# LariWa/Fractal-Image-Compression

Measured on NVIDIA B200. Metric: encode_evals_per_s, higher is better.
Workload: dtype u8

## Files before the change

### fractal-image-compression_b200/csrc/fic_search_umma.cu

```cuda
#include <cuda_fp16.h>

#include <cmath>
#include <mutex>
#include <tuple>
#include <vector>

#include "fic_device.cuh"

namespace fic {

namespace {

constexpr int kTileN = 128;
constexpr int kBlockM = 128;
constexpr int kAccs = 4;
constexpr int kRowsPerSB = kBlockM * kAccs;
constexpr int kEpiWarps = 16;
constexpr int kThreads = (4 + kEpiWarps) * 32;
constexpr int kChunksPerTile = kTileN / 32;
constexpr int kBoundBytes = kChunksPerTile * 2 * 4 + 16 + kChunksPerTile * 4;
constexpr int kNormOff = kChunksPerTile * 2 * 4 + 16;
constexpr int kFlagLists = 2;
constexpr int kFlagCap = 32;
constexpr float kOneMinusEps = 1.0f - 1.9073486328125e-06f;

template <int B, bool F16>
struct Cfg;
template <>
struct Cfg<8, false> {
    static constexpr int n = 64;
    static constexpr int NB = 4;
    static constexpr bool KSPLIT = false;
    static constexpr int KS_A = 3;
    static constexpr int KS_B = 5;
    static constexpr int NS = 5;
    static constexpr int NSTAGE = 7;
    __host__ __device__ static constexpr int amap(int s) { return s < 4 ? (s & 1) : 2; }
    __host__ __device__ static constexpr bool is_l_slice(int s) { return s == 2 || s == 3; }
};
template <>
struct Cfg<4, false> {
    static constexpr int n = 16;
    static constexpr int NB = 4;
    static constexpr bool KSPLIT = false;
    static constexpr int KS_A = 2;
    static constexpr int KS_B = 2;
    static constexpr int NS = 2;
    static constexpr int NSTAGE = 8;
    __host__ __device__ static constexpr int amap(int s) { return s; }
    __host__ __device__ static constexpr bool is_l_slice(int) { return false; }
};
template <>
struct Cfg<16, false> {
    static constexpr int n = 256;
    static constexpr int NB = 4;
    static constexpr bool KSPLIT = true;
    static constexpr int KS_P0 = 9, KS_P1 = 8;
    static constexpr int KS_A = 9;
    static constexpr int KS_B = 17;
    static constexpr int NS = 17;
    static constexpr int NSTAGE = 2;
    __host__ __device__ static constexpr int amap(int s) { return s < 16 ? (s & 7) : 8; }
    __host__ __device__ static constexpr bool is_l_slice(int s) { return s >= 8 && s < 16; }
};
template <>
struct Cfg<8, true> {
    static constexpr int n = 64;
    static constexpr int NB = 4;
    static constexpr bool KSPLIT = false;
    static constexpr int KS_A = 4;
    static constexpr int KS_B = 4;
    static constexpr int NS = 4;
    static constexpr int NSTAGE = 8;
    __host__ __device__ static constexpr int amap(int s) { return s; }
    __host__ __device__ static constexpr bool is_l_slice(int) { return false; }
};
template <>
struct Cfg<4, true> {
    static constexpr int n = 16;
    static constexpr int NB = 4;
    static constexpr bool KSPLIT = false;
    static constexpr int KS_A = 1;
    static constexpr int KS_B = 1;
    static constexpr int NS = 1;
    static constexpr int NSTAGE = 8;
    __host__ __device__ static constexpr int amap(int s) { return s; }
    __host__ __device__ static constexpr bool is_l_slice(int) { return false; }
};

template <>
struct Cfg<16, true> {
    static constexpr int n = 256;
    static constexpr int NB = 2;
    static constexpr bool KSPLIT = true;
    static constexpr int KS_P0 = 8, KS_P1 = 8;
    static constexpr int KS_A = 16;
    static constexpr int KS_B = 16;
    static constexpr int NS = 16;
    static constexpr int NSTAGE = 2;
    __host__ __device__ static constexpr int amap(int s) { return s; }
    __host__ __device__ static constexpr bool is_l_slice(int) { return false; }
};

template <class C>
constexpr int ksplit_p0()
{
    if constexpr (C::KSPLIT) return C::KS_P0;
    else return C::KS_B;
}

template <int B, bool F16>
struct Lay {
    using C = Cfg<B, F16>;
    static constexpr int SBO_A = C::KS_A * 256;
    static constexpr int A_BLOCK_BYTES = (kBlockM / 8) * SBO_A;
    static constexpr int ROWS_SB = C::NB * kBlockM;
    static constexpr int A_SB_BYTES = C::NB * A_BLOCK_BYTES;
    static constexpr int KS0 = ksplit_p0<C>();
    static constexpr int SBO_B = KS0 * 256;
    static constexpr int SBO_P1 = (C::KS_B - KS0) * 256;
    static constexpr int B_OP_BYTES = (kTileN / 8) * SBO_B;
    static constexpr int P0_BYTES = B_OP_BYTES + kBoundBytes;
    static constexpr int P1_BYTES = (kTileN / 8) * SBO_P1;
    static constexpr int B_TILE_BYTES = P0_BYTES + P1_BYTES;
    static constexpr int SLOT_BYTES = C::KSPLIT ? ((P0_BYTES + 127) / 128) * 128 : B_TILE_BYTES;
    static constexpr int PAIR_P0_BYTES = B_OP_BYTES / 2, PAIR_P1_BYTES = P1_BYTES / 2;
    static constexpr int PAIR_SLOT_BYTES = PAIR_P0_BYTES > PAIR_P1_BYTES ? PAIR_P0_BYTES : PAIR_P1_BYTES;
    static constexpr int PAIR_STAGES = (C::NSTAGE * SLOT_BYTES) / PAIR_SLOT_BYTES < 12 ? (C::NSTAGE * SLOT_BYTES) / PAIR_SLOT_BYTES : 12;
    static constexpr int BAR_BYTES = 512;
    static constexpr int SMEM_BYTES = A_SB_BYTES + C::NSTAGE * SLOT_BYTES + 1024  + BAR_BYTES  +
                                      kRowsPerSB * 4 ;
};

__device__ __noinline__ float flag_threshold(float lb, float tie_abs)
{
    const float rad = lb * lb * kOneMinusEps - tie_abs;
    return rad > 0.0f ? sqrtf(rad) : -1.0f;
}

struct RowFilter { float thresh, lbmax; int cnt; };
__device__ __noinline__ RowFilter flag_chunk(RowFilter st, float lb, float ub, float tie_abs, int2 *list, int chunk_id,
                                             uint32_t sh_lb, int share)
{
    if (st.cnt < kFlagCap) list[st.cnt] = make_int2(chunk_id, __float_as_int(ub));
    st.cnt++;
    if (lb > st.lbmax) {
        st.lbmax = lb;
        if (share)
            asm volatile("red.shared.max.u32 [%0], %1;" ::"r"(sh_lb), "r"(__float_as_uint(lb)) : "memory");
        const float rad = lb * lb * kOneMinusEps - tie_abs;
        st.thresh = rad > 0.0f ? sqrtf(rad) : -1.0f;
    }
    return st;
}


__host__ __device__ __forceinline__ int64_t sweep_to_sorted(int64_t pos, uint32_t mult, int64_t nch)
{
    const uint64_t chunk = (uint64_t)pos >> 5;
    return (int64_t)(((chunk * (uint64_t)mult) % (uint64_t)nch) * 32 + ((uint64_t)pos & 31));
}

__global__ void k_umma_sortkeys(const int32_t *__restrict__ dsum, const int32_t *__restrict__ dsq, int n,
                                int64_t ND, uint32_t *__restrict__ keys, int32_t *__restrict__ vals)
{
    int64_t j = (int64_t)blockIdx.x * blockDim.x + threadIdx.x;
    if (j >= ND) return;
    int dmean;
    keys[j] = (uint32_t)dom_var(dsum[j], dsq[j], n, &dmean);
    vals[j] = (int32_t)j;
}


constexpr int kSortSub = 512;

__global__ void __launch_bounds__(256) k_sort_hist(const uint32_t *__restrict__ keys, int64_t n, int shift, int64_t nwarps,
                                                   uint32_t *__restrict__ hist)
{
    __shared__ uint32_t s_h[8][256];
    const int warp = threadIdx.x >> 5, lane = threadIdx.x & 31;
    const int64_t gw = (int64_t)blockIdx.x * 8 + warp;
    for (int d = lane; d < 256; d += 32) s_h[warp][d] = 0;
    __syncwarp();
    if (gw < nwarps) {
        const int64_t a = gw * kSortSub, b = a + kSortSub < n ? a + kSortSub : n;
        for (int64_t i = a + lane; i < b; i += 32) atomicAdd(&s_h[warp][(keys[i] >> shift) & 255u], 1u);
        __syncwarp();
        for (int d = lane; d < 256; d += 32) hist[(int64_t)d * nwarps + gw] = s_h[warp][d];
    }
}

__global__ void __launch_bounds__(256) k_sort_scan_rows(uint32_t *__restrict__ hist, int64_t nwarps, uint32_t *__restrict__ totals)
{
    __shared__ uint32_t s_warp[8];
    __shared__ uint32_t s_carry;
    uint32_t *row = hist + (int64_t)blockIdx.x * nwarps;
    const int warp = threadIdx.x >> 5, lane = threadIdx.x & 31;
    if (threadIdx.x == 0) s_carry = 0;
    __syncthreads();
    for (int64_t base = 0; base < nwarps; base += 256) {
        const int64_t i = base + threadIdx.x;
        const uint32_t c = i < nwarps ? row[i] : 0u;
        uint32_t incl = c;
        for (int o = 1; o < 32; o <<= 1) {
            const uint32_t v = __shfl_up_sync(0xffffffffu, incl, o);
            if (lane >= o) incl += v;
        }
        if (lane == 31) s_warp[warp] = incl;
        __syncthreads();
        uint32_t before = s_carry;
        for (int w = 0; w < warp; w++) before += s_warp[w];
        if (i < nwarps) row[i] = before + incl - c;
        __syncthreads();
        if (threadIdx.x == 255) s_carry = before + incl;
        __syncthreads();
    }
    if (threadIdx.x == 0) totals[blockIdx.x] = s_carry;
}

__global__ void __launch_bounds__(256) k_sort_scatter(const uint32_t *__restrict__ keys, const int32_t *__restrict__ vals,
                                                      uint32_t *__restrict__ keys_out, int32_t *__restrict__ vals_out, int64_t n,
                                                      int shift, int64_t nwarps, const uint32_t *__restrict__ hist,
                                                      const uint32_t *__restrict__ totals)
{
    __shared__ uint32_t s_digit[256];
    __shared__ uint32_t s_base[8][256];
    const int warp = threadIdx.x >> 5, lane = threadIdx.x & 31;
    const int64_t gw = (int64_t)blockIdx.x * 8 + warp;
    {
        const uint32_t c = totals[threadIdx.x];
        uint32_t incl = c;
        for (int o = 1; o < 32; o <<= 1) {
            const uint32_t v = __shfl_up_sync(0xffffffffu, incl, o);
            if (lane >= o) incl += v;
        }
        s_digit[threadIdx.x] = incl - c;
        if (lane == 31) s_base[0][warp] = incl;
        __syncthreads();
        uint32_t before = 0;
        for (int w = 0; w < warp; w++) before += s_base[0][w];
        __syncthreads();
        s_digit[threadIdx.x] += before;
        __syncthreads();
    }
    if (gw >= nwarps) return;
    for (int d = lane; d < 256; d += 32) s_base[warp][d] = s_digit[d] + hist[(int64_t)d * nwarps + gw];
    __syncwarp();
    const int64_t a = gw * kSortSub, b = a + kSortSub < n ? a + kSortSub : n;
    for (int64_t i0 = a; i0 < b; i0 += 32) {
        const int64_t i = i0 + lane;
        const bool live = i < b;
        const uint32_t k = live ? keys[i] : 0u;
        const int32_t v = live ? vals[i] : 0;
        const uint32_t d = live ? ((k >> shift) & 255u) : 256u + lane;
        const unsigned peers = __match_any_sync(0xffffffffu, d);
        const int rank = __popc(peers & ((1u << lane) - 1u));
        uint32_t base = 0;
        if (live) base = s_base[warp][d];
        __syncwarp();
        if (live) {
            keys_out[base + rank] = k;
            vals_out[base + rank] = v;
            if (rank == 0) s_base[warp][d] = base + __popc(peers);
        }
        __syncwarp();
    }
}

inline size_t sort_hist_bytes(int64_t n) { return (size_t)256 * (size_t)((n + kSortSub - 1) / kSortSub + 1) * 4; }

inline int launch_sort_pairs(uint32_t *keys0, int32_t *vals0, uint32_t *keys1, int32_t *vals1, uint32_t *hist, int64_t n, cudaStream_t s)
{
    const int64_t nwarps = (n + kSortSub - 1) / kSortSub;
    const unsigned blocks = (unsigned)((nwarps + 7) / 8);
    uint32_t *totals = hist + 256 * nwarps;
    uint32_t *kin = keys0, *kout = keys1;
    int32_t *vin = vals0, *vout = vals1;
    for (int pass = 0; pass < 3; pass++) {
        k_sort_hist<<<blocks, 256, 0, s>>>(kin, n, 8 * pass, nwarps, hist);
        k_sort_scan_rows<<<256, 256, 0, s>>>(hist, nwarps, totals);
        k_sort_scatter<<<blocks, 256, 0, s>>>(kin, vin, kout, vout, n, 8 * pass, nwarps, hist, totals);
        uint32_t *tk = kin; kin = kout; kout = tk;
        int32_t *tv = vin; vin = vout; vout = tv;
    }
    return 9;
}


__device__ __forceinline__ uint32_t pack4(int a, int b, int c, int d)
{
    return (uint32_t)(a & 0xff) | ((uint32_t)(b & 0xff) << 8) | ((uint32_t)(c & 0xff) << 16) | ((uint32_t)(d & 0xff) << 24);
}

template <int n>
__host__ __device__ __forceinline__ int64_t raw_offset(int64_t pos, int c)
{
    return (pos >> 5) * (32 * n) + c * 512 + (pos & 31) * 16;
}

__device__ __forceinline__ uint32_t pack_h2(int lo, int hi)
{
    const __half2 v = __halves2half2(__int2half_rn(lo), __int2half_rn(hi));
    return *(const uint32_t *)&v;
}

template <int B, bool F16>
__global__ void __launch_bounds__(128)
k_umma_pack_domains(const uint8_t *__restrict__ dec, const int32_t *__restrict__ dsum,
                    const int32_t *__restrict__ dsq, const int32_t *__restrict__ perm, uint8_t *__restrict__ opB,
                    int32_t *__restrict__ pos_dom, int4 *__restrict__ pos_info,
                    uint8_t *__restrict__ pos_raw, int64_t *__restrict__ dom0_pos,
                    Geom g, int64_t ntiles, uint32_t mult)
{
    using L = Lay<B, F16>;
    constexpr int n = Cfg<B, F16>::n;
    const int64_t pos = (int64_t)blockIdx.x * blockDim.x + threadIdx.x;
    const int64_t tile = pos / kTileN;
    const int row = (int)(pos % kTileN);
    const int64_t sp = sweep_to_sorted(pos, mult, ntiles * kChunksPerTile);
    constexpr bool KSPLIT = Cfg<B, F16>::KSPLIT;
    uint8_t *blob = opB + tile * L::B_TILE_BYTES;
    uint8_t *rowp = blob + (row >> 3) * L::SBO_B + (row & 7) * 16;
    uint8_t *rowp1 = blob + L::P0_BYTES + (row >> 3) * L::SBO_P1 + (row & 7) * 16;
    constexpr int NCH = L::KS0 * 2;
    constexpr int NCH1 = (Cfg<B, F16>::KS_B - L::KS0) * 2;
    float rsd_hi = 0.0f, rsd_lo = __int_as_float(0x7f800000);
    int any_l = 0;
    if (sp >= g.ND) {
#pragma unroll
        for (int c = 0; c < NCH; c++) *(uint4 *)(rowp + c * 128) = make_uint4(0, 0, 0, 0);
#pragma unroll
        for (int c = 0; c < NCH1; c++) *(uint4 *)(rowp1 + c * 128) = make_uint4(0, 0, 0, 0);
        pos_dom[pos] = -1;
        pos_info[pos] = make_int4(-1, 0, 0, 0);
    } else {
        const int64_t j = perm[sp];
        const int gx = (int)(j % g.dpw), gy = (int)(j / g.dpw);
        const uint8_t *p = dec + (int64_t)(gy * g.step) * g.sw + gx * g.step;
        int dmean;
        const int varD = dom_var(dsum[j], dsq[j], n, &dmean);
        constexpr int PCH = n / 16;
        const int sgn = (!F16 && dmean == 0) ? -1 : 1;
        const bool wide8 = B == 8 && (g.sw & 7) == 0;
        const int col8 = (gx * g.step) & 7;
#pragma unroll
        for (int c = 0; c < PCH; c++) {
            int dv[16];
            uint32_t raw[4];
            if (wide8) {
#pragma unroll
                for (int r2 = 0; r2 < 2; r2++) {
                    const uint8_t *q = p + (int64_t)(c * 2 + r2) * g.sw - col8;
                    const uint2 lo = __ldg((const uint2 *)q);
                    uint2 hi = lo;
                    if (col8) hi = __ldg((const uint2 *)(q + 8));
                    const uint32_t sh = (uint32_t)(col8 & 3) * 8u;
                    const bool up = col8 >= 4;
                    raw[2 * r2] = __funnelshift_r(up ? lo.y : lo.x, up ? hi.x : lo.y, sh);
                    raw[2 * r2 + 1] = __funnelshift_r(up ? hi.x : lo.y, up ? hi.y : hi.x, sh);
                }
            }
#pragma unroll
            for (int w = 0; w < 4; w++) {
                const int k = c * 16 + w * 4;
                const uint8_t *q = p + (int64_t)(k / B) * g.sw + (k % B);
                if (B == 16) raw[w] = __ldg((const uint32_t *)q);
                else if (B == 8) {
                    if (!wide8) raw[w] = (uint32_t)__ldg((const uint16_t *)q) | ((uint32_t)__ldg((const uint16_t *)(q + 2)) << 16);
                } else raw[w] = (uint32_t)__ldg(q) | ((uint32_t)__ldg(q + 1) << 8) | ((uint32_t)__ldg(q + 2) << 16) | ((uint32_t)__ldg(q + 3) << 24);
#pragma unroll
                for (int e = 0; e < 4; e++) dv[w * 4 + e] = sgn * ((int)((raw[w] >> (8 * e)) & 0xffu) - dmean);
            }
            *(uint4 *)(pos_raw + raw_offset<n>(pos, c)) = make_uint4(raw[0], raw[1], raw[2], raw[3]);
            if (F16) {
                *(uint4 *)(rowp + (2 * c) * 128) =
                    make_uint4(pack_h2(dv[0], dv[1]), pack_h2(dv[2], dv[3]), pack_h2(dv[4], dv[5]), pack_h2(dv[6], dv[7]));
                *(uint4 *)(rowp + (2 * c + 1) * 128) = make_uint4(pack_h2(dv[8], dv[9]), pack_h2(dv[10], dv[11]),
                                                                  pack_h2(dv[12], dv[13]), pack_h2(dv[14], dv[15]));
            } else {
                uint32_t hw[4], lw[4];
#pragma unroll
                for (int w = 0; w < 4; w++) {
                    int hv[4], lv[4];
#pragma unroll
                    for (int e = 0; e < 4; e++) {
                        hv[e] = max(-128, min(127, dv[w * 4 + e]));
                        lv[e] = dv[w * 4 + e] - hv[e];
                        any_l |= lv[e];
                    }
                    hw[w] = pack4(hv[0], hv[1], hv[2], hv[3]);
                    lw[w] = pack4(lv[0], lv[1], lv[2], lv[3]);
                }
                *(uint4 *)(rowp + c * 128) = make_uint4(hw[0], hw[1], hw[2], hw[3]);
                if (KSPLIT) *(uint4 *)(rowp1 + c * 128) = make_uint4(lw[0], lw[1], lw[2], lw[3]);
                else *(uint4 *)(rowp + (PCH + c) * 128) = make_uint4(lw[0], lw[1], lw[2], lw[3]);
            }
        }
        if (!F16) {
            const int alpha = sgn * (dsum[j] - n * dmean);
            const int a1 = alpha / 3, a2 = (alpha - a1) / 2, a3 = alpha - a1 - a2;
            constexpr int ACH = KSPLIT ? PCH : 2 * PCH;
            *(uint4 *)(rowp + ACH * 128) = make_uint4(
                (uint32_t)((-a1) & 0xff) | ((uint32_t)((-a2) & 0xff) << 8) | ((uint32_t)((-a3) & 0xff) << 16), 0, 0, 0);
            *(uint4 *)(rowp + (ACH + 1) * 128) = make_uint4(0, 0, 0, 0);
        }
        pos_dom[pos] = (int32_t)j;
        pos_info[pos] = make_int4((int32_t)j, varD, dsum[j], 0);
        if (j == 0) *dom0_pos = pos;
        if (varD > 0) {
            float r = __double2float_rn(__ddiv_rn(1.0, __dsqrt_rn((double)varD)));
            rsd_hi = r * (1.0f + 4.76837158203125e-07f);
            rsd_lo = r * (1.0f - 4.76837158203125e-07f);
        }
    }
    for (int o = 16; o > 0; o >>= 1) {
        rsd_hi = fmaxf(rsd_hi, __shfl_xor_sync(0xffffffffu, rsd_hi, o));
        rsd_lo = fminf(rsd_lo, __shfl_xor_sync(0xffffffffu, rsd_lo, o));
    }
    if ((threadIdx.x & 31) == 0) {
        if (rsd_hi == 0.0f) rsd_lo = 0.0f;
        *(float2 *)(blob + L::B_OP_BYTES + (row >> 5) * 8) = make_float2(rsd_hi, rsd_lo);
    }
    const int tile_has_l = __syncthreads_or(any_l != 0);
    if (threadIdx.x == 0) *(uint4 *)(blob + L::B_OP_BYTES + kChunksPerTile * 8) = make_uint4((uint32_t)tile_has_l, 0, 0, 0);
}

template <int B, bool F16>
__global__ void __launch_bounds__(128)
k_umma_pack_ranges(const uint8_t *__restrict__ src, const int32_t *__restrict__ rsum, uint8_t *__restrict__ opA,
                   int32_t *__restrict__ vRout, Geom g, int64_t j0, int64_t j1, int64_t rows_padded)
{
    using L = Lay<B, F16>;
    constexpr int n = Cfg<B, F16>::n;
    int64_t i = (int64_t)blockIdx.x * blockDim.x + threadIdx.x;
    if (i >= rows_padded) return;
    int64_t sb = i / L::ROWS_SB;
    int rr = (int)(i % L::ROWS_SB);
    int blk = rr / kBlockM, row = rr % kBlockM;
    uint8_t *rowp = opA + sb * L::A_SB_BYTES + blk * L::A_BLOCK_BYTES + (row >> 3) * L::SBO_A + (row & 7) * 16;
    constexpr int NCH = Cfg<B, F16>::KS_A * 2;
    const int64_t j = j0 + i / g.n_iso;
    const int kiso = (int)(i % g.n_iso);
    if (j >= j1) {
#pragma unroll
        for (int c = 0; c < NCH; c++) *(uint4 *)(rowp + c * 128) = make_uint4(0, 0, 0, 0);
        vRout[i] = 0;
        return;
    }
    int xr = (int)(j % g.rpw), yr = (int)(j / g.rpw);
    const uint8_t *p = src + (int64_t)(yr * B) * g.W + xr * B;
    int rmean;
    vRout[i] = centred_sum(rsum[j], n, &rmean);
    constexpr int PCH = n / 16;
#pragma unroll
    for (int c = 0; c < PCH; c++) {
        uint32_t w4[4];
#pragma unroll
        for (int w = 0; w < 4; w++) {
            int k = c * 16 + w * 4;
            if (kiso == 0) {
                w4[w] = *(const uint32_t *)(p + (int64_t)(k / B) * g.W + (k % B));
            } else {
                w4[w] = 0;
#pragma unroll
                for (int e = 0; e < 4; e++) {
                    int ry, rx;
                    iso_map(iso_inverse(kiso), B, (k + e) / B, (k + e) % B, &ry, &rx);
                    w4[w] |= (uint32_t)p[(int64_t)ry * g.W + rx] << (8 * e);
                }
            }
        }
        if (F16) {
            uint32_t hw[8];
#pragma unroll
            for (int w = 0; w < 4; w++) {
                hw[2 * w] = pack_h2((int)(w4[w] & 0xff) - rmean, (int)((w4[w] >> 8) & 0xff) - rmean);
                hw[2 * w + 1] = pack_h2((int)((w4[w] >> 16) & 0xff) - rmean, (int)(w4[w] >> 24) - rmean);
            }
            *(uint4 *)(rowp + (2 * c) * 128) = make_uint4(hw[0], hw[1], hw[2], hw[3]);
            *(uint4 *)(rowp + (2 * c + 1) * 128) = make_uint4(hw[4], hw[5], hw[6], hw[7]);
        } else {
            uint4 v = make_uint4(w4[0], w4[1], w4[2], w4[3]);
            *(uint4 *)(rowp + c * 128) = v;
            if (B == 4) *(uint4 *)(rowp + (PCH + c) * 128) = v;
        }
    }
    if (!F16) {
        constexpr int XCH = (B == 4) ? 2 * PCH : PCH;
        *(uint4 *)(rowp + XCH * 128) = make_uint4((uint32_t)rmean | ((uint32_t)rmean << 8) | ((uint32_t)rmean << 16), 0, 0, 0);
        *(uint4 *)(rowp + (XCH + 1) * 128) = make_uint4(0, 0, 0, 0);
    }
}


__global__ void k_umma_sortkeys_rgb(const int32_t *__restrict__ dsum, int n, int64_t ND, uint32_t *__restrict__ keys,
                                    int32_t *__restrict__ vals)
{
    int64_t j = (int64_t)blockIdx.x * blockDim.x + threadIdx.x;
    if (j >= ND) return;
    int dm[3];
    const int vd = centred_sum_rgb(dsum, ND, j, n, dm);
    keys[j] = (uint32_t)(vd * vd);
    vals[j] = (int32_t)j;
}

template <int B>
__device__ __forceinline__ uint8_t *rgb_dom_piece(uint8_t *blob, int row, int c)
{
    using L = Lay<B, true>;
    constexpr int NCH0 = L::KS0 * 2;
    if (!Cfg<B, true>::KSPLIT || c < NCH0) return blob + (row >> 3) * L::SBO_B + (row & 7) * 16 + c * 128;
    return blob + L::P0_BYTES + (row >> 3) * L::SBO_P1 + (row & 7) * 16 + (c - NCH0) * 128;
}

template <int B>
__global__ void __launch_bounds__(128)
k_umma_pack_domains_rgb(const uint16_t *__restrict__ dec3, const int32_t *__restrict__ dsum,
                        const int32_t *__restrict__ perm, uint8_t *__restrict__ opB, int32_t *__restrict__ pos_dom,
                        int4 *__restrict__ pos_info, int64_t *__restrict__ dom0_pos, Geom g, int64_t ntiles, uint32_t mult)
{
    using L = Lay<B, true>;
    constexpr int n = B * B;
    const int64_t pos = (int64_t)blockIdx.x * blockDim.x + threadIdx.x;
    const int64_t tile = pos / kTileN;
    const int row = (int)(pos % kTileN);
    const int64_t sp = sweep_to_sorted(pos, mult, ntiles * kChunksPerTile);
    uint8_t *blob = opB + tile * L::B_TILE_BYTES;
    constexpr int NCH = n / 8;
    float rsd_hi = 0.0f, rsd_lo = __int_as_float(0x7f800000), norm = 0.0f;
    if (sp >= g.ND) {
#pragma unroll
        for (int c = 0; c < NCH; c++) *(uint4 *)rgb_dom_piece<B>(blob, row, c) = make_uint4(0, 0, 0, 0);
        pos_dom[pos] = -1;
        pos_info[pos] = make_int4(-1, 0, 0, 0);
    } else {
        const int64_t j = perm[sp];
        const int gx = (int)(j % g.dpw), gy = (int)(j / g.dpw);
        const uint16_t *p = dec3 + (int64_t)(gy * g.step) * g.sw + gx * g.step;
        int dm[3];
        const int vd = centred_sum_rgb(dsum, g.ND, j, n, dm);
        const int dmsum = dm[0] + dm[1] + dm[2];
        uint32_t sumsq = 0;
#pragma unroll
        for (int c = 0; c < NCH; c++) {
            int dv[8];
            const int k0 = c * 8;
            const uint16_t *q = p + (int64_t)(k0 / B) * g.sw + (k0 % B);
            if (B == 16) {
#pragma unroll
                for (int e = 0; e < 8; e += 4) {
                    const uint2 w = __ldg((const uint2 *)(q + e));
                    dv[e] = (int)(w.x & 0xffffu); dv[e + 1] = (int)(w.x >> 16);
                    dv[e + 2] = (int)(w.y & 0xffffu); dv[e + 3] = (int)(w.y >> 16);
                }
            } else if (B == 8) {
#pragma unroll
                for (int e = 0; e < 8; e += 2) {
                    const uint32_t w = __ldg((const uint32_t *)(q + e));
                    dv[e] = (int)(w & 0xffffu);
                    dv[e + 1] = (int)(w >> 16);
                }
            } else {
#pragma unroll
                for (int e = 0; e < 8; e++) {
                    const int k = k0 + e;
                    dv[e] = (int)__ldg(p + (int64_t)(k / B) * g.sw + (k % B));
                }
            }
#pragma unroll
            for (int e = 0; e < 8; e++) {
                dv[e] = vd != 0 ? dv[e] - dmsum : 0;
                sumsq += (uint32_t)(dv[e] * dv[e]);
            }
            *(uint4 *)rgb_dom_piece<B>(blob, row, c) =
                make_uint4(pack_h2(dv[0], dv[1]), pack_h2(dv[2], dv[3]), pack_h2(dv[4], dv[5]), pack_h2(dv[6], dv[7]));
        }
        pos_dom[pos] = (int32_t)j;
        pos_info[pos] = make_int4((int32_t)j, vd, 0, 0);
        if (j == 0) *dom0_pos = pos;
        if (vd > 0) {
            float r = __double2float_rn(__ddiv_rn(1.0, (double)vd));
            rsd_hi = r * (1.0f + 4.76837158203125e-07f);
            rsd_lo = r * (1.0f - 4.76837158203125e-07f);
        }
        norm = __fsqrt_ru((float)sumsq) * (1.0f + 2.384185791015625e-07f);
    }
    for (int o = 16; o > 0; o >>= 1) {
        rsd_hi = fmaxf(rsd_hi, __shfl_xor_sync(0xffffffffu, rsd_hi, o));
        rsd_lo = fminf(rsd_lo, __shfl_xor_sync(0xffffffffu, rsd_lo, o));
        norm = fmaxf(norm, __shfl_xor_sync(0xffffffffu, norm, o));
    }
    if ((threadIdx.x & 31) == 0) {
        if (rsd_hi == 0.0f) rsd_lo = 0.0f;
        *(float2 *)(blob + L::B_OP_BYTES + (row >> 5) * 8) = make_float2(rsd_hi, rsd_lo);
        *(float *)(blob + L::B_OP_BYTES + kNormOff + (row >> 5) * 4) = norm;
    }
    if (threadIdx.x == 0) *(uint4 *)(blob + L::B_OP_BYTES + kChunksPerTile * 8) = make_uint4(Cfg<B, true>::KSPLIT ? 1u : 0u, 0, 0, 0);
}

template <int B>
__global__ void __launch_bounds__(128)
k_umma_pack_ranges_rgb(const uint8_t *__restrict__ src, const int32_t *__restrict__ rsum, uint8_t *__restrict__ opA,
                       int32_t *__restrict__ vRout, float *__restrict__ nRout, Geom g, int64_t j0, int64_t j1, int64_t rows_padded)
{
    using L = Lay<B, true>;
    constexpr int n = B * B;
    int64_t i = (int64_t)blockIdx.x * blockDim.x + threadIdx.x;
    if (i >= rows_padded) return;
    int64_t sb = i / L::ROWS_SB;
    int rr = (int)(i % L::ROWS_SB);
    int blk = rr / kBlockM, row = rr % kBlockM;
    uint8_t *rowp = opA + sb * L::A_SB_BYTES + blk * L::A_BLOCK_BYTES + (row >> 3) * L::SBO_A + (row & 7) * 16;
    constexpr int NCH = n / 8;
    const int64_t j = j0 + i;
    if (j >= j1) {
#pragma unroll
        for (int c = 0; c < NCH; c++) *(uint4 *)(rowp + c * 128) = make_uint4(0, 0, 0, 0);
        vRout[i] = 0;
        if (nRout) nRout[i] = 0.0f;
        return;
    }
    const int xr = (int)(j % g.rpw), yr = (int)(j / g.rpw);
    const int64_t plane = (int64_t)g.W * g.H;
    const uint8_t *p = src + (int64_t)(yr * B) * g.W + xr * B;
    int rm[3];
    const int vR = centred_sum_rgb(rsum, g.NR, j, n, rm);
    const int rmsum = rm[0] + rm[1] + rm[2];
    uint32_t sumsq = 0;
#pragma unroll
    for (int c = 0; c < NCH; c++) {
        int rv[8];
#pragma unroll
        for (int e = 0; e < 8; e++) {
            const int k = c * 8 + e;
            const uint8_t *q = p + (int64_t)(k / B) * g.W + (k % B);
            rv[e] = (int)q[0] + (int)q[plane] + (int)q[2 * plane] - rmsum;
            sumsq += (uint32_t)(rv[e] * rv[e]);
        }
        *(uint4 *)(rowp + c * 128) =
            make_uint4(pack_h2(rv[0], rv[1]), pack_h2(rv[2], rv[3]), pack_h2(rv[4], rv[5]), pack_h2(rv[6], rv[7]));
    }
    vRout[i] = vR;
    if (nRout) nRout[i] = __fsqrt_ru((float)sumsq) * (1.0f + 2.384185791015625e-07f);
}


__device__ __forceinline__ uint32_t smem_u32(const void *p) { return (uint32_t)__cvta_generic_to_shared(p); }

__device__ __forceinline__ void mbar_init(uint32_t bar, uint32_t count)
{
    asm volatile("mbarrier.init.shared::cta.b64 [%0], %1;" ::"r"(bar), "r"(count));
}
__device__ __forceinline__ void mbar_arrive(uint32_t bar)
{
    asm volatile("mbarrier.arrive.shared::cta.b64 _, [%0];" ::"r"(bar) : "memory");
}
__device__ __forceinline__ void mbar_expect_tx(uint32_t bar, uint32_t bytes)
{
    asm volatile("mbarrier.arrive.expect_tx.shared::cta.b64 _, [%0], %1;" ::"r"(bar), "r"(bytes) : "memory");
}
__device__ __forceinline__ uint32_t mbar_try_wait(uint32_t bar, uint32_t parity)
{
    uint32_t ok;
    asm volatile(
        "{\n\t.reg .pred p;\n\t"
        "mbarrier.try_wait.parity.shared::cta.b64 p, [%1], %2;\n\t"
        "selp.u32 %0, 1, 0, p;\n\t}"
        : "=r"(ok)
        : "r"(bar), "r"(parity)
        : "memory");
    return ok;
}
__device__ __noinline__ void mbar_timeout(volatile int *status, int code)
{
    if (status) {
        *status = code;
        __threadfence_system();
    }
    __trap();
}
__device__ __noinline__ void mbar_wait_slow(uint32_t bar, uint32_t parity, volatile int *status, int code)
{
    long long t0 = clock64();
    while (!mbar_try_wait(bar, parity)) {
        if (clock64() - t0 > 2000000000ll) mbar_timeout(status, code);
    }
}
__device__ __forceinline__ void mbar_wait(uint32_t bar, uint32_t parity, volatile int *status, int code)
{
    if (mbar_try_wait(bar, parity)) return;
    mbar_wait_slow(bar, parity, status, code);
}
__device__ __forceinline__ void bulk_g2s(uint32_t dst, const void *src, uint32_t bytes, uint32_t bar)
{
    asm volatile("cp.async.bulk.shared::cluster.global.mbarrier::complete_tx::bytes [%0], [%1], %2, [%3];" ::"r"(dst),
                 "l"(src), "r"(bytes), "r"(bar)
                 : "memory");
}
__device__ __forceinline__ uint32_t elect_one()
{
    uint32_t pred;
    asm volatile(
        "{\n\t.reg .pred p;\n\t.reg .b32 r;\n\t"
        "elect.sync r|p, 0xffffffff;\n\t"
        "selp.u32 %0, 1, 0, p;\n\t}"
        : "=r"(pred));
    return pred;
}
__device__ __forceinline__ void tc_fence_before() { asm volatile("tcgen05.fence::before_thread_sync;" ::: "memory"); }
__device__ __forceinline__ void tc_fence_after() { asm volatile("tcgen05.fence::after_thread_sync;" ::: "memory"); }
__device__ __forceinline__ void tc_commit(uint32_t bar)
{
    asm volatile("tcgen05.commit.cta_group::1.mbarrier::arrive::one.shared::cluster.b64 [%0];" ::"r"(bar) : "memory");
}
__device__ __forceinline__ void tc_mma_i8(uint32_t d_tmem, uint64_t adesc, uint64_t bdesc, uint32_t idesc, uint32_t acc)
{
    asm volatile(
        "{\n\t.reg .pred p;\n\tsetp.ne.b32 p, %4, 0;\n\t"
        "tcgen05.mma.cta_group::1.kind::i8 [%0], %1, %2, %3, p;\n\t}" ::"r"(d_tmem),
        "l"(adesc), "l"(bdesc), "r"(idesc), "r"(acc)
        : "memory");
}
__device__ __forceinline__ void tc_mma_f16(uint32_t d_tmem, uint64_t adesc, uint64_t bdesc, uint32_t idesc, uint32_t acc)
{
    asm volatile(
        "{\n\t.reg .pred p;\n\tsetp.ne.b32 p, %4, 0;\n\t"
        "tcgen05.mma.cta_group::1.kind::f16 [%0], %1, %2, %3, p;\n\t}" ::"r"(d_tmem),
        "l"(adesc), "l"(bdesc), "r"(idesc), "r"(acc)
        : "memory");
}
__device__ __forceinline__ uint32_t cluster_ctarank()
{
    uint32_t r;
    asm volatile("mov.u32 %0, %%cluster_ctarank;" : "=r"(r));
    return r;
}
__device__ __forceinline__ void cluster_sync_all()
{
    asm volatile("barrier.cluster.arrive.release.aligned;\n\tbarrier.cluster.wait.acquire.aligned;" ::: "memory");
}
__device__ __forceinline__ uint32_t mapa_u32(uint32_t saddr, uint32_t rank)
{
    uint32_t r;
    asm volatile("mapa.shared::cluster.u32 %0, %1, %2;" : "=r"(r) : "r"(saddr), "r"(rank));
    return r;
}
__device__ __forceinline__ void mbar_arrive_cluster(uint32_t cluster_addr)
{
    asm volatile("mbarrier.arrive.shared::cluster.b64 _, [%0];" ::"r"(cluster_addr) : "memory");
}
__device__ __forceinline__ void tc_commit2(uint32_t bar, uint32_t mask)
{
    asm volatile("tcgen05.commit.cta_group::2.mbarrier::arrive::one.shared::cluster.multicast::cluster.b64 [%0], %1;" ::"r"(bar),
                 "h"((uint16_t)mask)
                 : "memory");
}
__device__ __forceinline__ void tc_mma2_i8(uint32_t d_tmem, uint64_t adesc, uint64_t bdesc, uint32_t idesc, uint32_t acc)
{
    asm volatile(
        "{\n\t.reg .pred p;\n\tsetp.ne.b32 p, %4, 0;\n\t"
        "tcgen05.mma.cta_group::2.kind::i8 [%0], %1, %2, %3, p;\n\t}" ::"r"(d_tmem),
        "l"(adesc), "l"(bdesc), "r"(idesc), "r"(acc)
        : "memory");
}
__device__ __forceinline__ void tc_mma2_f16(uint32_t d_tmem, uint64_t adesc, uint64_t bdesc, uint32_t idesc, uint32_t acc)
{
    asm volatile(
        "{\n\t.reg .pred p;\n\tsetp.ne.b32 p, %4, 0;\n\t"
        "tcgen05.mma.cta_group::2.kind::f16 [%0], %1, %2, %3, p;\n\t}" ::"r"(d_tmem),
        "l"(adesc), "l"(bdesc), "r"(idesc), "r"(acc)
        : "memory");
}
__device__ __forceinline__ void tmem_ld32(uint32_t taddr, uint32_t (&v)[32])
{
    asm volatile(
        "tcgen05.ld.sync.aligned.32x32b.x32.b32 "
        "{%0, %1, %2, %3, %4, %5, %6, %7, %8, %9, %10, %11, %12, %13, %14, %15, "
        "%16, %17, %18, %19, %20, %21, %22, %23, %24, %25, %26, %27, %28, %29, %30, %31}, [%32];"
        : "=r"(v[0]), "=r"(v[1]), "=r"(v[2]), "=r"(v[3]), "=r"(v[4]), "=r"(v[5]), "=r"(v[6]), "=r"(v[7]),
          "=r"(v[8]), "=r"(v[9]), "=r"(v[10]), "=r"(v[11]), "=r"(v[12]), "=r"(v[13]), "=r"(v[14]), "=r"(v[15]),
          "=r"(v[16]), "=r"(v[17]), "=r"(v[18]), "=r"(v[19]), "=r"(v[20]), "=r"(v[21]), "=r"(v[22]), "=r"(v[23]),
          "=r"(v[24]), "=r"(v[25]), "=r"(v[26]), "=r"(v[27]), "=r"(v[28]), "=r"(v[29]), "=r"(v[30]), "=r"(v[31])
        : "r"(taddr)
        : "memory");
}
__device__ __forceinline__ void sts_u32(uint32_t saddr, uint32_t v)
{
    asm volatile("st.shared.u32 [%0], %1;" ::"r"(saddr), "r"(v) : "memory");
}
__device__ __forceinline__ uint32_t lds_volatile_u32(uint32_t saddr)
{
    uint32_t v;
    asm volatile("ld.volatile.shared.u32 %0, [%1];" : "=r"(v) : "r"(saddr) : "memory");
    return v;
}
__device__ __forceinline__ void pin_order(uint32_t (&v)[32])
{
    asm volatile(""
                 : "+r"(v[0]), "+r"(v[1]), "+r"(v[2]), "+r"(v[3]), "+r"(v[4]), "+r"(v[5]), "+r"(v[6]), "+r"(v[7]), "+r"(v[8]),
                   "+r"(v[9]), "+r"(v[10]), "+r"(v[11]), "+r"(v[12]), "+r"(v[13]), "+r"(v[14]), "+r"(v[15]), "+r"(v[16]),
                   "+r"(v[17]), "+r"(v[18]), "+r"(v[19]), "+r"(v[20]), "+r"(v[21]), "+r"(v[22]), "+r"(v[23]), "+r"(v[24]),
                   "+r"(v[25]), "+r"(v[26]), "+r"(v[27]), "+r"(v[28]), "+r"(v[29]), "+r"(v[30]), "+r"(v[31])
                 :
                 : "memory");
}
__device__ __forceinline__ void tmem_ld_wait() { asm volatile("tcgen05.wait::ld.sync.aligned;" ::: "memory"); }
__device__ __forceinline__ int dp4a_uu(uint32_t a_u8x4, uint32_t b_u8x4, int c)
{
    int d;
    asm("dp4a.u32.u32 %0, %1, %2, %3;" : "=r"(d) : "r"(a_u8x4), "r"(b_u8x4), "r"(c));
    return d;
}

__device__ __forceinline__ uint64_t make_desc(uint32_t saddr, uint32_t lbo_bytes, uint32_t sbo_bytes)
{
    return (uint64_t)((saddr >> 4) & 0x3fff) | ((uint64_t)((lbo_bytes >> 4) & 0x3fff) << 16) |
           ((uint64_t)((sbo_bytes >> 4) & 0x3fff) << 32) | ((uint64_t)1 << 46);
}

constexpr uint32_t kIdesc = (2u << 4) | (0u << 7) | (1u << 10) | ((uint32_t)(kTileN >> 3) << 17) |
                            ((uint32_t)(kBlockM >> 4) << 24);
constexpr uint32_t kIdescF16 = (1u << 4) | (0u << 7) | (0u << 10) | ((uint32_t)(kTileN >> 3) << 17) |
                               ((uint32_t)(kBlockM >> 4) << 24);
constexpr uint32_t kIdescPair = (2u << 4) | (0u << 7) | (1u << 10) | ((uint32_t)(kTileN >> 3) << 17) |
                                ((uint32_t)((2 * kBlockM) >> 4) << 24);
constexpr uint32_t kIdescF16Pair = (1u << 4) | (0u << 7) | (0u << 10) | ((uint32_t)(kTileN >> 3) << 17) |
                                   ((uint32_t)((2 * kBlockM) >> 4) << 24);


template <int B, bool F16, bool PAIR>
__host__ __device__ constexpr int epi_of() { return (!F16 || B == 16) ? 0 : ((B == 4 || PAIR) ? 3 : 2); }

template <int B, bool F16, bool PAIR, bool DUMP>
__global__ void __launch_bounds__(kThreads, 1)
k_umma_search(const uint8_t *__restrict__ opA, const uint8_t *__restrict__ opB, const int32_t *__restrict__ vRarr,
              const float *__restrict__ nRarr, int2 *__restrict__ flag_list, int32_t *__restrict__ flag_cnt, uint32_t *__restrict__ row_lb, int n_sb,
              int n_chunks, int ntiles, int iso_shift, int64_t rows_padded, int32_t *__restrict__ dump, int64_t dump_ld, volatile int *status)
{
    using C = Cfg<B, F16>;
    using L = Lay<B, F16>;
    static_assert(!PAIR || F16 || C::KSPLIT, "CTA pairs: kind::f16, or the K-split configurations (B = 16)");
    constexpr int EPI = DUMP ? 0 : epi_of<B, F16, PAIR>();
    constexpr int NISS = (PAIR && !C::KSPLIT) ? 2 : 1;
    constexpr int NSTAGE = PAIR ? L::PAIR_STAGES : C::NSTAGE;
    constexpr int SLOT = PAIR ? L::PAIR_SLOT_BYTES : L::SLOT_BYTES;
    extern __shared__ __align__(1024) uint8_t smem_raw[];
    uint8_t *smem = (uint8_t *)(((uintptr_t)smem_raw + 1023) & ~(uintptr_t)1023);
    uint8_t *sA = smem;
    uint8_t *sB = smem + L::A_SB_BYTES;
    uint64_t *bars = (uint64_t *)(sB + C::NSTAGE * L::SLOT_BYTES);
    uint32_t bar0 = smem_u32(bars);
    asm volatile("" : "+r"(bar0));
    auto BAR_B_FULL = [&](int s) { return bar0 + 8u * s; };
    auto BAR_B_EMPTY = [&](int s) { return bar0 + 8u * (NSTAGE + s); };
    auto BAR_T_FULL = [&](int q) { return bar0 + 8u * (2 * NSTAGE + q); };
    auto BAR_T_EMPTY = [&](int q) { return bar0 + 8u * (2 * NSTAGE + kAccs + q); };
    const uint32_t BAR_A_FULL = bar0 + 8u * (2 * NSTAGE + 2 * kAccs);
    const uint32_t BAR_A_EMPTY = BAR_A_FULL + 8u;
    uint32_t *tmem_slot = (uint32_t *)(bars + 2 * NSTAGE + 2 * kAccs + 2);
    const uint32_t s_has_l = bar0 + 400u;
    uint32_t *s_lb = (uint32_t *)((uint8_t *)bars + L::BAR_BYTES);

    const int warp = threadIdx.x >> 5, lane = threadIdx.x & 31;
    const uint32_t rank = PAIR ? cluster_ctarank() : 0u;
    const int u_first = PAIR ? (int)(blockIdx.x >> 1) : (int)blockIdx.x, u_step = PAIR ? (int)(gridDim.x >> 1) : (int)gridDim.x;
    const int n_sbu = PAIR ? (n_sb >> 1) : n_sb;

    if (warp == 1 && lane == 0) {
        const uint32_t both = (PAIR && rank == 0) ? 2u : 1u;
        for (int s = 0; s < NSTAGE; s++) {
            mbar_init(BAR_B_FULL(s), both);
            mbar_init(BAR_B_EMPTY(s), NISS);
        }
        for (int q = 0; q < kAccs; q++) {
            mbar_init(BAR_T_FULL(q), 1);
            mbar_init(BAR_T_EMPTY(q), both * (kEpiWarps / kAccs));
        }
        mbar_init(BAR_A_FULL, both);
        mbar_init(BAR_A_EMPTY, NISS);
        asm volatile("fence.mbarrier_init.release.cluster;" ::: "memory");
    }
    if (warp == 2) {
        if (PAIR) {
            asm volatile("tcgen05.alloc.cta_group::2.sync.aligned.shared::cta.b32 [%0], %1;" ::"r"(smem_u32(tmem_slot)), "r"(512u) : "memory");
            asm volatile("tcgen05.relinquish_alloc_permit.cta_group::2.sync.aligned;" ::: "memory");
        } else {
            asm volatile("tcgen05.alloc.cta_group::1.sync.aligned.shared::cta.b32 [%0], %1;" ::"r"(smem_u32(tmem_slot)), "r"(512u) : "memory");
            asm volatile("tcgen05.relinquish_alloc_permit.cta_group::1.sync.aligned;" ::: "memory");
        }
    }
    tc_fence_before();
    if (PAIR) cluster_sync_all();
    else __syncthreads();
    tc_fence_after();
    const uint32_t tmem_base = *tmem_slot;

    const int n_units = n_sbu * n_chunks;

    if (warp == 0) {
        if (lane == 0) {
            uint32_t stage = 0, phase = 0, a_phase = 0;
            for (int u = u_first; u < n_units; u += u_step) {
                int sb = PAIR ? 2 * (u % n_sbu) + (int)rank : u % n_sbu, ch = u / n_sbu;
                int t0 = (int)((int64_t)ch * ntiles / n_chunks), t1 = (int)((int64_t)(ch + 1) * ntiles / n_chunks);
                mbar_wait(BAR_A_EMPTY, a_phase ^ 1, status, 1);
                mbar_expect_tx(BAR_A_FULL, L::A_SB_BYTES);
                bulk_g2s(smem_u32(sA), opA + (int64_t)sb * L::A_SB_BYTES, L::A_SB_BYTES, BAR_A_FULL);
                for (int t = t0; t < t1; t++) {
                    const uint8_t *blob = opB + (int64_t)t * L::B_TILE_BYTES;
                    if (C::KSPLIT && PAIR) {
                        const uint32_t has_l = __ldg((const uint32_t *)(blob + L::B_OP_BYTES + kChunksPerTile * 8));
                        mbar_wait(BAR_B_EMPTY(stage), phase ^ 1, status, 2);
                        sts_u32(s_has_l + 4u * stage, has_l);
                        mbar_expect_tx(BAR_B_FULL(stage), L::PAIR_P0_BYTES);
                        bulk_g2s(smem_u32(sB + stage * SLOT), blob + rank * L::PAIR_P0_BYTES, L::PAIR_P0_BYTES, BAR_B_FULL(stage));
                        if (++stage == NSTAGE) { stage = 0; phase ^= 1; }
                        if (has_l) {
                            mbar_wait(BAR_B_EMPTY(stage), phase ^ 1, status, 2);
                            mbar_expect_tx(BAR_B_FULL(stage), L::PAIR_P1_BYTES);
                            bulk_g2s(smem_u32(sB + stage * SLOT), blob + L::P0_BYTES + rank * L::PAIR_P1_BYTES, L::PAIR_P1_BYTES, BAR_B_FULL(stage));
                            if (++stage == NSTAGE) { stage = 0; phase ^= 1; }
                        }
                    } else if (C::KSPLIT) {
                        mbar_wait(BAR_B_EMPTY(stage), phase ^ 1, status, 2);
                        mbar_expect_tx(BAR_B_FULL(stage), L::P0_BYTES);
                        bulk_g2s(smem_u32(sB + stage * L::SLOT_BYTES), blob, L::P0_BYTES, BAR_B_FULL(stage));
                        if (++stage == NSTAGE) { stage = 0; phase ^= 1; }
                        const uint32_t has_l = __ldg((const uint32_t *)(blob + L::B_OP_BYTES + kChunksPerTile * 8));
                        if (has_l) {
                            mbar_wait(BAR_B_EMPTY(stage), phase ^ 1, status, 2);
                            mbar_expect_tx(BAR_B_FULL(stage), L::P1_BYTES);
                            bulk_g2s(smem_u32(sB + stage * L::SLOT_BYTES), blob + L::P0_BYTES, L::P1_BYTES, BAR_B_FULL(stage));
                            if (++stage == NSTAGE) { stage = 0; phase ^= 1; }
                        }
                    } else if (PAIR) {
                        mbar_wait(BAR_B_EMPTY(stage), phase ^ 1, status, 2);
                        mbar_expect_tx(BAR_B_FULL(stage), SLOT);
                        bulk_g2s(smem_u32(sB + stage * SLOT), blob + rank * SLOT, SLOT, BAR_B_FULL(stage));
                        if (++stage == NSTAGE) { stage = 0; phase ^= 1; }
                    } else {
                        mbar_wait(BAR_B_EMPTY(stage), phase ^ 1, status, 2);
                        mbar_expect_tx(BAR_B_FULL(stage), L::B_TILE_BYTES);
                        bulk_g2s(smem_u32(sB + stage * L::SLOT_BYTES), blob, L::B_TILE_BYTES, BAR_B_FULL(stage));
                        if (++stage == NSTAGE) { stage = 0; phase ^= 1; }
                    }
                }
                a_phase ^= 1;
            }
        }
        __syncwarp();
    } else if (PAIR && (warp == 1 || (warp == 3 && !C::KSPLIT))) {
        if constexpr (PAIR && C::KSPLIT) {
            if (rank == 0) {
                uint32_t stage = 0, phase = 0, a_phase = 0, t_phase = 0;
                const uint32_t elected = elect_one();
                const uint64_t a_desc0 = make_desc(smem_u32(sA), 128, L::SBO_A);
                for (int u = u_first; u < n_units; u += u_step) {
                    int ch = u / n_sbu;
                    int t0 = (int)((int64_t)ch * ntiles / n_chunks), t1 = (int)((int64_t)(ch + 1) * ntiles / n_chunks);
                    mbar_wait(BAR_A_FULL, a_phase, status, 3);
                    for (int t = t0; t < t1; t++) {
                        mbar_wait(BAR_B_FULL(stage), phase, status, 4);
                        tc_fence_after();
                        const uint32_t has_l = lds_volatile_u32(s_has_l + 4u * stage);
                        const uint64_t b0 = make_desc(smem_u32(sB + stage * SLOT), 128, L::SBO_B);
#pragma unroll
                        for (int q = 0; q < C::NB; q++) {
                            mbar_wait(BAR_T_EMPTY(q), ((t_phase >> q) & 1) ^ 1, status, 5);
                            tc_fence_after();
                            if (elected) {
#pragma unroll
                                for (int s = 0; s < L::KS0; s++) {
                                    const uint64_t ad = a_desc0 + (uint64_t)((q * L::A_BLOCK_BYTES + s * 256) >> 4);
                                    if (F16) tc_mma2_f16(tmem_base + q * kTileN, ad, b0 + (uint64_t)((s * 256) >> 4), kIdescF16Pair, s > 0 ? 1u : 0u);
                                    else tc_mma2_i8(tmem_base + q * kTileN, ad, b0 + (uint64_t)((s * 256) >> 4), kIdescPair, s > 0 ? 1u : 0u);
                                }
                                if (!has_l) tc_commit2(BAR_T_FULL(q), 3u);
                            }
                            __syncwarp();
                            t_phase ^= 1u << q;
                        }
                        if (elected) tc_commit2(BAR_B_EMPTY(stage), 3u);
                        __syncwarp();
                        if (++stage == NSTAGE) { stage = 0; phase ^= 1; }
                        if (has_l) {
                            mbar_wait(BAR_B_FULL(stage), phase, status, 4);
                            tc_fence_after();
                            const uint64_t b1 = make_desc(smem_u32(sB + stage * SLOT), 128, L::SBO_P1);
#pragma unroll
                            for (int q = 0; q < C::NB; q++) {
                                if (elected) {
#pragma unroll
                                    for (int s = 0; s < C::KS_B - L::KS0; s++) {
                                        const int sa = F16 ? L::KS0 + s : s;
                                        const uint64_t ad = a_desc0 + (uint64_t)((q * L::A_BLOCK_BYTES + sa * 256) >> 4);
                                        if (F16) tc_mma2_f16(tmem_base + q * kTileN, ad, b1 + (uint64_t)((s * 256) >> 4), kIdescF16Pair, 1u);
                                        else tc_mma2_i8(tmem_base + q * kTileN, ad, b1 + (uint64_t)((s * 256) >> 4), kIdescPair, 1u);
                                    }
                                    tc_commit2(BAR_T_FULL(q), 3u);
                                }
                                __syncwarp();
                            }
                            if (elected) tc_commit2(BAR_B_EMPTY(stage), 3u);
                            __syncwarp();
                            if (++stage == NSTAGE) { stage = 0; phase ^= 1; }
                        }
                    }
                    if (elected) tc_commit2(BAR_A_EMPTY, 3u);
                    __syncwarp();
                    a_phase ^= 1;
                }
            } else {
                if (lane == 0) {
                    uint32_t stage = 0, phase = 0, a_phase = 0;
                    const uint32_t ra_full = mapa_u32(BAR_A_FULL, 0);
                    for (int u = u_first; u < n_units; u += u_step) {
                        int ch = u / n_sbu;
                        int t0 = (int)((int64_t)ch * ntiles / n_chunks), t1 = (int)((int64_t)(ch + 1) * ntiles / n_chunks);
                        mbar_wait(BAR_A_FULL, a_phase, status, 3);
                        mbar_arrive_cluster(ra_full);
                        for (int t = t0; t < t1; t++) {
                            mbar_wait(BAR_B_FULL(stage), phase, status, 4);
                            const uint32_t has_l = lds_volatile_u32(s_has_l + 4u * stage);
                            mbar_arrive_cluster(mapa_u32(BAR_B_FULL(stage), 0));
                            if (++stage == NSTAGE) { stage = 0; phase ^= 1; }
                            if (has_l) {
                                mbar_wait(BAR_B_FULL(stage), phase, status, 4);
                                mbar_arrive_cluster(mapa_u32(BAR_B_FULL(stage), 0));
                                if (++stage == NSTAGE) { stage = 0; phase ^= 1; }
                            }
                        }
                        a_phase ^= 1;
                    }
                }
                __syncwarp();
            }
        } else if constexpr (PAIR) {
            if (rank == 0) {
                const int qi = warp >> 1;
                uint32_t stage = 0, phase = 0, a_phase = 0, t_phase = 0;
                const uint32_t elected = elect_one();
                const uint64_t a_desc0 = make_desc(smem_u32(sA), 128, L::SBO_A);
                const uint64_t b_desc0 = make_desc(smem_u32(sB), 128, L::SBO_B);
                for (int u = u_first; u < n_units; u += u_step) {
                    int ch = u / n_sbu;
                    int t0 = (int)((int64_t)ch * ntiles / n_chunks), t1 = (int)((int64_t)(ch + 1) * ntiles / n_chunks);
                    mbar_wait(BAR_A_FULL, a_phase, status, 3);
                    for (int t = t0; t < t1; t++) {
                        mbar_wait(BAR_B_FULL(stage), phase, status, 4);
                        tc_fence_after();
                        const uint64_t b_desc = b_desc0 + (uint64_t)((stage * SLOT) >> 4);
#pragma unroll
                        for (int k = 0; k < 2; k++) {
                            const int q = qi + 2 * k;
                            mbar_wait(BAR_T_EMPTY(q), ((t_phase >> k) & 1) ^ 1, status, 5);
                            tc_fence_after();
                            if (elected) {
#pragma unroll
                                for (int s = 0; s < C::NS; s++) {
                                    const uint64_t ad = a_desc0 + (uint64_t)((q * L::A_BLOCK_BYTES + C::amap(s) * 256) >> 4);
                                    tc_mma2_f16(tmem_base + q * kTileN, ad, b_desc + (uint64_t)((s * 256) >> 4), kIdescF16Pair, s > 0 ? 1u : 0u);
                                }
                                tc_commit2(BAR_T_FULL(q), 3u);
                                if (k == 1) tc_commit2(BAR_B_EMPTY(stage), 3u);
                            }
                            __syncwarp();
                            t_phase ^= 1u << k;
                        }
                        if (++stage == NSTAGE) { stage = 0; phase ^= 1; }
                    }
                    if (elected) tc_commit2(BAR_A_EMPTY, 3u);
                    __syncwarp();
                    a_phase ^= 1;
                }
            } else if (warp == 1) {
                if (lane == 0) {
                    uint32_t stage = 0, phase = 0, a_phase = 0;
                    const uint32_t ra_full = mapa_u32(BAR_A_FULL, 0);
                    for (int u = u_first; u < n_units; u += u_step) {
                        int ch = u / n_sbu;
                        int t0 = (int)((int64_t)ch * ntiles / n_chunks), t1 = (int)((int64_t)(ch + 1) * ntiles / n_chunks);
                        mbar_wait(BAR_A_FULL, a_phase, status, 3);
                        mbar_arrive_cluster(ra_full);
                        for (int t = t0; t < t1; t++) {
                            mbar_wait(BAR_B_FULL(stage), phase, status, 4);
                            mbar_arrive_cluster(mapa_u32(BAR_B_FULL(stage), 0));
                            if (++stage == NSTAGE) { stage = 0; phase ^= 1; }
                        }
                        a_phase ^= 1;
                    }
                }
                __syncwarp();
            }
        }
    } else if (warp == 1) {
        uint32_t stage = 0, phase = 0, a_phase = 0, t_phase = 0;
        const uint32_t elected = elect_one();
        const uint64_t a_desc0 = make_desc(smem_u32(sA), 128, L::SBO_A);
        const uint64_t b_desc0 = make_desc(smem_u32(sB), 128, L::SBO_B);
        for (int u = u_first; u < n_units; u += u_step) {
            int ch = u / n_sbu;
            int t0 = (int)((int64_t)ch * ntiles / n_chunks), t1 = (int)((int64_t)(ch + 1) * ntiles / n_chunks);
            mbar_wait(BAR_A_FULL, a_phase, status, 3);
            for (int t = t0; t < t1; t++) {
                mbar_wait(BAR_B_FULL(stage), phase, status, 4);
                tc_fence_after();
                const uint32_t has_l = *(volatile const uint32_t *)(sB + stage * L::SLOT_BYTES + L::B_OP_BYTES + kChunksPerTile * 8);
                if (C::KSPLIT) {
                    const uint64_t b0 = make_desc(smem_u32(sB + stage * L::SLOT_BYTES), 128, L::SBO_B);
#pragma unroll
                    for (int q = 0; q < C::NB; q++) {
                        mbar_wait(BAR_T_EMPTY(q), ((t_phase >> q) & 1) ^ 1, status, 5);
                        tc_fence_after();
                        if (elected) {
#pragma unroll
                            for (int s = 0; s < L::KS0; s++) {
                                const uint64_t ad = a_desc0 + (uint64_t)((q * L::A_BLOCK_BYTES + s * 256) >> 4);
                                if (F16) tc_mma_f16(tmem_base + q * kTileN, ad, b0 + (uint64_t)((s * 256) >> 4), kIdescF16, s > 0 ? 1u : 0u);
                                else tc_mma_i8(tmem_base + q * kTileN, ad, b0 + (uint64_t)((s * 256) >> 4), kIdesc, s > 0 ? 1u : 0u);
                            }
                            if (!has_l) tc_commit(BAR_T_FULL(q));
                        }
                        __syncwarp();
                        t_phase ^= 1u << q;
                    }
                    if (elected) tc_commit(BAR_B_EMPTY(stage));
                    __syncwarp();
                    if (++stage == NSTAGE) { stage = 0; phase ^= 1; }
                    if (has_l) {
                        mbar_wait(BAR_B_FULL(stage), phase, status, 4);
                        tc_fence_after();
                        const uint64_t b1 = make_desc(smem_u32(sB + stage * L::SLOT_BYTES), 128, L::SBO_P1);
#pragma unroll
                        for (int q = 0; q < C::NB; q++) {
                            if (elected) {
#pragma unroll
                                for (int s = 0; s < C::KS_B - L::KS0; s++) {
                                    const int sa = F16 ? L::KS0 + s : s;
                                    const uint64_t ad = a_desc0 + (uint64_t)((q * L::A_BLOCK_BYTES + sa * 256) >> 4);
                                    if (F16) tc_mma_f16(tmem_base + q * kTileN, ad, b1 + (uint64_t)((s * 256) >> 4), kIdescF16, 1u);
                                    else tc_mma_i8(tmem_base + q * kTileN, ad, b1 + (uint64_t)((s * 256) >> 4), kIdesc, 1u);
                                }
                                tc_commit(BAR_T_FULL(q));
                            }
                            __syncwarp();
                        }
                        if (elected) tc_commit(BAR_B_EMPTY(stage));
                        __syncwarp();
                        if (++stage == NSTAGE) { stage = 0; phase ^= 1; }
                    }
                    continue;
                }
                const uint64_t b_desc = b_desc0 + (uint64_t)((stage * L::SLOT_BYTES) >> 4);
#pragma unroll
                for (int q = 0; q < C::NB; q++) {
                    mbar_wait(BAR_T_EMPTY(q), ((t_phase >> q) & 1) ^ 1, status, 5);
                    tc_fence_after();
                    if (elected) {
#pragma unroll
                        for (int s = 0; s < C::NS; s++) {
                            if (C::is_l_slice(s) && !has_l) continue;
                            const uint64_t ad = a_desc0 + (uint64_t)((q * L::A_BLOCK_BYTES + C::amap(s) * 256) >> 4);
                            const uint64_t bd = b_desc + (uint64_t)((s * 256) >> 4);
                            if (F16) tc_mma_f16(tmem_base + q * kTileN, ad, bd, kIdescF16, s > 0 ? 1u : 0u);
                            else tc_mma_i8(tmem_base + q * kTileN, ad, bd, kIdesc, s > 0 ? 1u : 0u);
                        }
                        tc_commit(BAR_T_FULL(q));
                    }
                    __syncwarp();
                    t_phase ^= 1u << q;
                }
                if (elected) tc_commit(BAR_B_EMPTY(stage));
                __syncwarp();
                if (++stage == NSTAGE) { stage = 0; phase ^= 1; }
            }
            if (elected) tc_commit(BAR_A_EMPTY);
            __syncwarp();
            a_phase ^= 1;
        }
    } else if (warp >= 4) {
        const int e = warp - 4;
        const int lq = e & 3, q = e >> 2;
        const uint32_t ta = tmem_base + ((uint32_t)(lq * 32) << 16) + q * kTileN;
        uint32_t tf_phase = 0;
        const uint32_t bar_hand_back = PAIR ? mapa_u32(BAR_T_EMPTY(q), 0) : BAR_T_EMPTY(q);
        auto hand_back = [&]() {
            if (PAIR) mbar_arrive_cluster(bar_hand_back);
            else mbar_arrive(bar_hand_back);
        };
        constexpr bool SLACK = B == 16 && F16;
        const int n_units_mine = q < C::NB ? n_units : 0;
        for (int u = u_first; u < n_units_mine; u += u_step) {
            int sb = PAIR ? 2 * (u % n_sbu) + (int)rank : u % n_sbu, ch = u / n_sbu;
            int t0 = (int)((int64_t)ch * ntiles / n_chunks), t1 = (int)((int64_t)(ch + 1) * ntiles / n_chunks);
            const int64_t row = (int64_t)sb * L::ROWS_SB + q * kBlockM + lq * 32 + lane;
            const int vR = vRarr[row];
            const float nR = SLACK ? nRarr[row] : 0.0f;
            RowFilter st;
            st.thresh = (vR == 0) ? __int_as_float(0x7f800000) : -1.0f;
            st.lbmax = 0.0f;
            st.cnt = 0;
            const float tie_abs = (float)(vR * vR) * 4.76837158203125e-07f;
            const uint32_t sh_lb = smem_u32(s_lb + q * kBlockM + (((lq * 32 + lane) >> iso_shift) << iso_shift));
            if (iso_shift) {
                sts_u32(sh_lb, 0u);
                __syncwarp();
            }
            if (ch > 0 && vR != 0) {
                const float seed = __uint_as_float(*(volatile const uint32_t *)(row_lb + ((row >> iso_shift) << iso_shift)));
                if (seed > 0.0f) {
                    st.lbmax = seed;
                    st.thresh = flag_threshold(seed, tie_abs);
                }
            }
            int2 *const list0 = flag_list + (((int64_t)ch * rows_padded + row) * kFlagLists) * kFlagCap;
            int cnt0 = 0, cnt1 = 0;
            for (int t = t0; t < t1; t++) {
                const float4 *gb = (const float4 *)(opB + (int64_t)t * L::B_TILE_BYTES + L::B_OP_BYTES);
                const float4 bnd01 = __ldg(gb), bnd23 = __ldg(gb + 1);
                float4 bndn = make_float4(0.0f, 0.0f, 0.0f, 0.0f);
                if (SLACK) bndn = __ldg(gb + 3);
                mbar_wait(BAR_T_FULL(q), tf_phase, status, 7);
                tc_fence_after();
                if (iso_shift) {
                    const float other = __uint_as_float(lds_volatile_u32(sh_lb));
                    if (other > st.lbmax) {
                        st.lbmax = other;
                        st.thresh = flag_threshold(other, tie_abs);
                    }
                }
                if constexpr (EPI != 0) {
                    uint32_t v[32];
                    float Mc[kChunksPerTile];
                    tmem_ld32(ta, v);
                    tmem_ld_wait();
                    pin_order(v);
                    auto test = [&](int c) {
                        const float rhi = c == 0 ? bnd01.x : (c == 1 ? bnd01.z : (c == 2 ? bnd23.x : bnd23.z));
                        const float rlo = c == 0 ? bnd01.y : (c == 1 ? bnd01.w : (c == 2 ? bnd23.y : bnd23.w));
                        const float ub = Mc[c] * rhi;
                        if (ub > st.thresh) {
                            st.cnt = c < 2 ? cnt0 : cnt1;
                            st = flag_chunk(st, Mc[c] * rlo, ub, tie_abs, list0 + (c >> 1) * kFlagCap, t * kChunksPerTile + c, sh_lb, iso_shift ? 1 : 0);
                            if (c < 2) cnt0 = st.cnt;
                            else cnt1 = st.cnt;
                        }
                    };
#pragma unroll
                    for (int c = 0; c < kChunksPerTile; c++) {
                        auto av = [&](int k) { return fabsf(__uint_as_float(v[k])); };
                        float l[11];
#pragma unroll
                        for (int i = 0; i < 10; i++) l[i] = fmaxf(fmaxf(av(3 * i), av(3 * i + 1)), av(3 * i + 2));
                        l[10] = fmaxf(av(30), av(31));
                        if (c + 1 < kChunksPerTile) {
                            uint32_t next = ta + (c + 1) * 32;
                            asm volatile("" : "+r"(next) : "f"(l[0]), "f"(l[1]), "f"(l[2]), "f"(l[3]), "f"(l[4]), "f"(l[5]), "f"(l[6]),
                                         "f"(l[7]), "f"(l[8]), "f"(l[9]), "f"(l[10]));
                            tmem_ld32(next, v);
                        }
                        asm volatile("" : "+f"(l[0]), "+f"(l[1]), "+f"(l[2]), "+f"(l[3]), "+f"(l[4]), "+f"(l[5]), "+f"(l[6]), "+f"(l[7]),
                                     "+f"(l[8]), "+f"(l[9]), "+f"(l[10]));
                        const float m0 = fmaxf(fmaxf(l[0], l[1]), l[2]), m1 = fmaxf(fmaxf(l[3], l[4]), l[5]);
                        const float m2 = fmaxf(fmaxf(l[6], l[7]), l[8]), m3 = fmaxf(fmaxf(l[9], l[10]), m0);
                        Mc[c] = fmaxf(fmaxf(m1, m2), m3);
                        if (EPI == 2) test(c);
                        if (c + 1 < kChunksPerTile) {
                            tmem_ld_wait();
                            pin_order(v);
                            if (c + 1 == kChunksPerTile - 1) {
                                tc_fence_before();
                                __syncwarp();
                                if (lane == 0) hand_back();
                                if (EPI == 3) {
                                    asm volatile("" : "+f"(Mc[0]), "+f"(Mc[1]), "+f"(Mc[2]) : : "memory");
                                    test(0);
                                    test(1);
                                    test(2);
                                }
                            }
                        }
                    }
                    if (EPI == 3) test(kChunksPerTile - 1);
                } else {
#pragma unroll
                for (int c = 0; c < kChunksPerTile; c++) {
                    uint32_t v[32];
                    tmem_ld32(ta + c * 32, v);
                    tmem_ld_wait();
                    if (c == kChunksPerTile - 1) {
                        tc_fence_before();
                        __syncwarp();
                        if (lane == 0) hand_back();
                    }
                    float M;
                    if (F16) {
                        auto av = [&](int k) { return fabsf(__uint_as_float(v[k])); };
                        float c4[4];
#pragma unroll
                        for (int i = 0; i < 4; i++) {
                            c4[i] = fmaxf(fmaxf(av(8 * i), av(8 * i + 1)), av(8 * i + 2));
                            c4[i] = fmaxf(c4[i], fmaxf(av(8 * i + 3), av(8 * i + 4)));
                            c4[i] = fmaxf(c4[i], fmaxf(av(8 * i + 5), av(8 * i + 6)));
                        }
                        const float m01 = fmaxf(fmaxf(c4[0], c4[1]), av(7));
                        const float m23 = fmaxf(fmaxf(c4[2], c4[3]), av(15));
                        M = fmaxf(fmaxf(fmaxf(m01, m23), av(23)), av(31));
                    } else {
                        int mx0 = 0, mn0 = 0, mx1 = 0, mn1 = 0;
#pragma unroll
                        for (int k = 0; k < 32; k += 4) {
                            mx0 = max(mx0, max((int)v[k], (int)v[k + 1]));
                            mn0 = min(mn0, min((int)v[k], (int)v[k + 1]));
                            mx1 = max(mx1, max((int)v[k + 2], (int)v[k + 3]));
                            mn1 = min(mn1, min((int)v[k + 2], (int)v[k + 3]));
                        }
                        M = __int2float_rn(max(max(mx0, mx1), -min(mn0, mn1)));
                    }
                    if (DUMP) {
#pragma unroll
                        for (int k = 0; k < 32; k++) {
                            int iv = (int)v[k];
                            if (F16) {
                                const float f = __uint_as_float(v[k]);
                                iv = (f == rintf(f) && fabsf(f) < 2.0e9f) ? (int)f : (int)0x80000000;
                            }
                            dump[row * dump_ld + (int64_t)t * kTileN + c * 32 + k] = iv;
                        }
                    }
                    const float rhi = c == 0 ? bnd01.x : (c == 1 ? bnd01.z : (c == 2 ? bnd23.x : bnd23.z));
                    const float rlo = c == 0 ? bnd01.y : (c == 1 ? bnd01.w : (c == 2 ? bnd23.y : bnd23.w));
                    float Mu = M, Ml = M;
                    if (SLACK) {
                        const float pn = nR * (c == 0 ? bndn.x : (c == 1 ? bndn.y : (c == 2 ? bndn.z : bndn.w)));
                        if (pn >= 16777216.0f) {
                            const float sl = pn * 6.0e-5f;
                            Mu = M + sl;
                            Ml = fmaxf(M - sl, 0.0f);
                        }
                    }
                    const float ub = Mu * rhi;
                    if (ub > st.thresh) {
                        st.cnt = c < 2 ? cnt0 : cnt1;
                        st = flag_chunk(st, Ml * rlo, ub, tie_abs, list0 + (c >> 1) * kFlagCap, t * kChunksPerTile + c, sh_lb, iso_shift ? 1 : 0);
                        if (c < 2) cnt0 = st.cnt;
                        else cnt1 = st.cnt;
                    }
                }
                }
                tf_phase ^= 1;
            }
            flag_cnt[((int64_t)ch * rows_padded + row) * 2] = cnt0;
            flag_cnt[((int64_t)ch * rows_padded + row) * 2 + 1] = cnt1;
            if (st.lbmax > 0.0f) atomicMax(row_lb + ((row >> iso_shift) << iso_shift), __float_as_uint(st.lbmax));
        }
    }

    tc_fence_before();
    if (PAIR) cluster_sync_all();
    else __syncthreads();
    if (warp == 2) {
        tc_fence_after();
        if (PAIR) asm volatile("tcgen05.dealloc.cta_group::2.sync.aligned.b32 %0, %1;" ::"r"(tmem_base), "r"(512u) : "memory");
        else asm volatile("tcgen05.dealloc.cta_group::1.sync.aligned.b32 %0, %1;" ::"r"(tmem_base), "r"(512u) : "memory");
    }
}


template <bool F16, int N>
__global__ void __launch_bounds__(128, 1) k_mma_peak(int iters, uint32_t seed)
{
    extern __shared__ __align__(1024) uint8_t smem_raw[];
    uint8_t *smem = (uint8_t *)(((uintptr_t)smem_raw + 1023) & ~(uintptr_t)1023);
    uint8_t *sA = smem;
    uint8_t *sB = smem + 4096;
    uint64_t *bar = (uint64_t *)(smem + 4096 + 8192);
    uint32_t *tmem_slot = (uint32_t *)(bar + 1);
    const int warp = threadIdx.x >> 5;
    for (int i = threadIdx.x; i < (4096 + 8192) / 4; i += blockDim.x) {
        uint32_t x = (uint32_t)i * 2654435761u + seed + blockIdx.x * 40503u;
        x ^= x >> 15; x *= 0x2c1b3c6du; x ^= x >> 12;
        if (F16) x &= 0x3fff3fffu;
        ((uint32_t *)smem)[i] = x;
    }
    if (threadIdx.x == 0) {
        mbar_init(smem_u32(bar), 1);
        asm volatile("fence.mbarrier_init.release.cluster;" ::: "memory");
    }
    asm volatile("fence.proxy.async.shared::cta;" ::: "memory");
    if (warp == 0) {
        asm volatile("tcgen05.alloc.cta_group::1.sync.aligned.shared::cta.b32 [%0], %1;" ::"r"(smem_u32(tmem_slot)),
                     "r"(512u)
                     : "memory");
        asm volatile("tcgen05.relinquish_alloc_permit.cta_group::1.sync.aligned;" ::: "memory");
    }
    tc_fence_before();
    __syncthreads();
    tc_fence_after();
    const uint32_t tmem_base = *tmem_slot;
    if (warp == 1) {
        const uint32_t elected = elect_one();
        const uint64_t ad = make_desc(smem_u32(sA), 128, 256);
        const uint64_t bd = make_desc(smem_u32(sB), 128, 256);
        constexpr uint32_t idesc = (F16 ? ((1u << 4) | (0u << 7) | (0u << 10)) : ((2u << 4) | (0u << 7) | (1u << 10))) |
                                   ((uint32_t)(N >> 3) << 17) | ((uint32_t)(128 >> 4) << 24);
        constexpr int NACC = 512 / N;
        if (elected) {
            for (int i = 0; i < iters; i++) {
                const uint32_t d = tmem_base + (uint32_t)(i & (NACC - 1)) * N;
                if (F16) tc_mma_f16(d, ad, bd, idesc, i >= NACC ? 1u : 0u);
                else tc_mma_i8(d, ad, bd, idesc, i >= NACC ? 1u : 0u);
            }
            tc_commit(smem_u32(bar));
        }
        __syncwarp();
        mbar_wait(smem_u32(bar), 0, nullptr, 9);
    }
    tc_fence_before();
    __syncthreads();
    if (warp == 0) {
        tc_fence_after();
        asm volatile("tcgen05.dealloc.cta_group::1.sync.aligned.b32 %0, %1;" ::"r"(tmem_base), "r"(512u) : "memory");
    }
}

template <bool F16>
__global__ void __launch_bounds__(128, 1) k_mma_peak_pair(int iters, uint32_t seed, uint32_t *out)
{
    extern __shared__ __align__(1024) uint8_t smem_raw[];
    uint8_t *smem = (uint8_t *)(((uintptr_t)smem_raw + 1023) & ~(uintptr_t)1023);
    uint8_t *sA = smem;
    uint8_t *sB = smem + 4096;
    uint64_t *bar = (uint64_t *)(smem + 4096 + 8192);
    uint32_t *tmem_slot = (uint32_t *)(bar + 1);
    const int warp = threadIdx.x >> 5;
    const uint32_t rank = cluster_ctarank();
    for (int i = threadIdx.x; i < (4096 + 8192) / 4; i += blockDim.x) {
        uint32_t x = (uint32_t)i * 2654435761u + seed + blockIdx.x * 40503u;
        x ^= x >> 15; x *= 0x2c1b3c6du; x ^= x >> 12;
        if (F16) x &= 0x3fff3fffu;
        ((uint32_t *)smem)[i] = x;
    }
    if (threadIdx.x == 0) {
        mbar_init(smem_u32(bar), 1);
        asm volatile("fence.mbarrier_init.release.cluster;" ::: "memory");
    }
    asm volatile("fence.proxy.async.shared::cta;" ::: "memory");
    if (warp == 0) {
        asm volatile("tcgen05.alloc.cta_group::2.sync.aligned.shared::cta.b32 [%0], %1;" ::"r"(smem_u32(tmem_slot)), "r"(256u) : "memory");
        asm volatile("tcgen05.relinquish_alloc_permit.cta_group::2.sync.aligned;" ::: "memory");
    }
    tc_fence_before();
    cluster_sync_all();
    tc_fence_after();
    const uint32_t tmem_base = *tmem_slot;
    if (threadIdx.x == 0 && out) out[blockIdx.x] = tmem_base;
    if (warp == 1) {
        if (rank == 0) {
            const uint32_t elected = elect_one();
            const uint64_t ad = make_desc(smem_u32(sA), 128, 256);
            const uint64_t bd = make_desc(smem_u32(sB), 128, 256);
            constexpr uint32_t idesc = (F16 ? ((1u << 4) | (0u << 7) | (0u << 10)) : ((2u << 4) | (0u << 7) | (1u << 10))) |
                                       ((uint32_t)(128 >> 3) << 17) | ((uint32_t)(256 >> 4) << 24);
            if (elected) {
                for (int i = 0; i < iters; i++) {
                    const uint32_t d = tmem_base + (uint32_t)(i & 1) * 128;
                    if (F16) tc_mma2_f16(d, ad, bd, idesc, i >= 2 ? 1u : 0u);
                    else tc_mma2_i8(d, ad, bd, idesc, i >= 2 ? 1u : 0u);
                }
                tc_commit2(smem_u32(bar), 3u);
            }
            __syncwarp();
        }
        mbar_wait(smem_u32(bar), 0, nullptr, 9);
    }
    tc_fence_before();
    cluster_sync_all();
    if (warp == 0) {
        tc_fence_after();
        asm volatile("tcgen05.dealloc.cta_group::2.sync.aligned.b32 %0, %1;" ::"r"(tmem_base), "r"(256u) : "memory");
    }
}


template <int B>
__device__ __forceinline__ int refine_kov(const uint32_t *rw, int rmean, int vR, const uint8_t *__restrict__ pos_raw,
                                          int64_t pos, int dsum)
{
    constexpr int n = B * B;
    int kov = 0;
#pragma unroll
    for (int c = 0; c < n / 16; c++) {
        const uint4 d = __ldg((const uint4 *)(pos_raw + raw_offset<n>(pos, c)));
        const uint4 r = *(const uint4 *)(rw + 4 * c);
        kov = dp4a_uu(r.x, d.x, kov);
        kov = dp4a_uu(r.y, d.y, kov);
        kov = dp4a_uu(r.z, d.z, kov);
        kov = dp4a_uu(r.w, d.w, kov);
    }
    return kov - (rmean * dsum + (dsum / n) * vR);
}

template <class F>
__device__ __forceinline__ void for_each_flagged(int lane, int64_t i, int64_t rows_padded, int n_chunks, int64_t npos,
                                                 const int2 *__restrict__ flag_list, const int32_t *__restrict__ flag_cnt,
                                                 float th, F &&consider)
{
    const int n_lists = kFlagLists * n_chunks;
    const int my_cnt = lane < n_lists ? flag_cnt[((int64_t)(lane / kFlagLists) * rows_padded + i) * kFlagLists + (lane % kFlagLists)] : 0;
    const bool overflow = __any_sync(0xffffffffu, my_cnt > kFlagCap);
    if (!overflow) {
        for (int lh = 0; lh < n_lists; lh++) {
            const int cnt = __shfl_sync(0xffffffffu, my_cnt, lh);
            if (cnt == 0) continue;
            const int2 *lst = flag_list + (((int64_t)(lh / kFlagLists) * rows_padded + i) * kFlagLists + (lh % kFlagLists)) * kFlagCap;
            const int2 mine = lane < cnt ? lst[lane] : make_int2(0, 0);
            unsigned live = __ballot_sync(0xffffffffu, lane < cnt && __int_as_float(mine.y) > th);
            while (live) {
                const int e = __ffs(live) - 1;
                live &= live - 1;
                consider((int64_t)__shfl_sync(0xffffffffu, mine.x, e) * 32 + lane);
            }
        }
    } else {
        for (int64_t pos = lane; pos < npos; pos += 32) consider(pos);
    }
}

template <int B>
__global__ void __launch_bounds__(128)
k_umma_refine(const uint8_t *__restrict__ src, const int32_t *__restrict__ rsum, const uint8_t *__restrict__ pos_raw,
              const int4 *__restrict__ pos_info,
              const int2 *__restrict__ flag_list, const int32_t *__restrict__ flag_cnt,
              const uint32_t *__restrict__ row_lb, int n_chunks,
              int64_t rows_padded, int64_t rows, int64_t npos, const int64_t *__restrict__ dom0_pos,
              int32_t *__restrict__ best, Geom g, int64_t j0)
{
    constexpr int n = B * B;
    constexpr int NW = n / 4;
    const int warp = threadIdx.x >> 5, lane = threadIdx.x & 31;
    const int64_t i = (int64_t)blockIdx.x * 4 + warp;
    if (i >= rows) return;
    const int64_t j = j0 + i;
    int rmean;
    const int vR = centred_sum(rsum[j], n, &rmean);
    if (vR == 0) {
        if (lane == 0) best[j] = 0;
        return;
    }
    const int xr = (int)(j % g.rpw), yr = (int)(j / g.rpw);
    constexpr bool RW_SMEM = B == 16;
    __shared__ __align__(16) uint32_t s_rw[RW_SMEM ? 4 : 1][RW_SMEM ? NW : 4];
    __align__(16) uint32_t rw_reg[RW_SMEM ? 4 : NW];
    const uint32_t *rw;
    if constexpr (RW_SMEM) {
        for (int w = lane; w < NW; w += 32) {
            const int k = 4 * w;
            s_rw[warp][w] = __ldg((const uint32_t *)(src + (int64_t)(yr * B + k / B) * g.W + xr * B + (k % B)));
        }
        __syncwarp();
        rw = s_rw[warp];
    } else {
#pragma unroll
        for (int w = 0; w < NW; w++) {
            const int k = 4 * w;
            rw_reg[w] = __ldg((const uint32_t *)(src + (int64_t)(yr * B + k / B) * g.W + xr * B + (k % B)));
        }
        rw = rw_reg;
    }
    float be = 10000000.0f;
    int bi = 0x7fffffff;
    const float tie_abs = (float)(vR * vR) * 4.76837158203125e-07f;
    float lb = __uint_as_float(row_lb[i]), th = lb > 0.0f ? flag_threshold(lb, tie_abs) : -1.0f;
    const float th_row = th;
    auto consider = [&](int64_t pos) {
        const int4 pi = __ldg(pos_info + pos);
        const int idx = pi.x;
        if (idx >= 0) {
            const int varD = pi.y;
            const int kov = refine_kov<B>(rw, rmean, vR, pos_raw, pos, pi.z);
            const float ax = varD > 0 ? fabsf((float)kov) * __frsqrt_rn((float)varD) : 0.0f;
            if (ax * (1.0f + 2.384185791015625e-07f) > th) {
                argmin_merge(be, bi, grey_error(kov, vR, __dsqrt_rn((double)varD)), idx);
                const float xlo = ax * (1.0f - 2.384185791015625e-07f);
                if (xlo > lb) { lb = xlo; th = flag_threshold(lb, tie_abs); }
            }
        }
    };
    if (lane == 0) consider(*dom0_pos);
    for_each_flagged(lane, i, rows_padded, n_chunks, npos, flag_list, flag_cnt, th_row, consider);
    warp_argmin(be, bi);
    if (lane == 0) best[j] = bi == 0x7fffffff ? 0 : bi;
}

template <int B>
__global__ void __launch_bounds__(128)
k_umma_refine_iso(const uint8_t *__restrict__ src, const int32_t *__restrict__ rsum, const uint8_t *__restrict__ pos_raw,
                  const int4 *__restrict__ pos_info, const int2 *__restrict__ flag_list,
                  const int32_t *__restrict__ flag_cnt, const uint32_t *__restrict__ row_lb, int n_chunks,
                  int64_t rows_padded, int64_t ranges, int64_t npos,
                  const int64_t *__restrict__ dom0_pos, int32_t *__restrict__ best, Geom g, int64_t j0)
{
    constexpr int n = B * B;
    constexpr int NW = n / 4;
    __shared__ uint8_t s_blk[4][n];
    const int warp = threadIdx.x >> 5, lane = threadIdx.x & 31;
    const int64_t r = (int64_t)blockIdx.x * 4 + warp;
    if (r >= ranges) return;
    const int64_t j = j0 + r;
    int rmean;
    const int vR = centred_sum(rsum[j], n, &rmean);
    if (vR == 0) {
        if (lane == 0) best[j] = 0;
        return;
    }
    const int xr = (int)(j % g.rpw), yr = (int)(j / g.rpw);
    for (int w = lane; w < NW; w += 32) {
        const int k = 4 * w;
        ((uint32_t *)s_blk[warp])[w] = __ldg((const uint32_t *)(src + (int64_t)(yr * B + k / B) * g.W + xr * B + (k % B)));
    }
    __syncwarp();
    __shared__ __align__(16) uint32_t s_rw[4][8][NW];
    for (int t = lane; t < 8 * NW; t += 32) {
        const int kiso = t / NW, w = t % NW;
        uint32_t word = 0;
#pragma unroll
        for (int e = 0; e < 4; e++) {
            int ry, rx;
            iso_map(iso_inverse(kiso), B, (4 * w + e) / B, (4 * w + e) % B, &ry, &rx);
            word |= (uint32_t)s_blk[warp][ry * B + rx] << (8 * e);
        }
        s_rw[warp][kiso][w] = word;
    }
    __syncwarp();
    const uint32_t *rw = s_rw[warp][0];
    auto build = [&](int kiso) { rw = s_rw[warp][kiso]; };
    float be = 10000000.0f;
    int bi = 0x7fffffff;
    const float tie_abs = (float)(vR * vR) * 4.76837158203125e-07f;
    float lb = __uint_as_float(row_lb[r * 8]), th = lb > 0.0f ? flag_threshold(lb, tie_abs) : -1.0f;
    const float th_row = th;
    auto consider = [&](int64_t pos, int kiso) {
        const int4 pi = __ldg(pos_info + pos);
        if (pi.x >= 0) {
            const int kov = refine_kov<B>(rw, rmean, vR, pos_raw, pos, pi.z);
            const float ax = pi.y > 0 ? fabsf((float)kov) * __frsqrt_rn((float)pi.y) : 0.0f;
            if (ax * (1.0f + 2.384185791015625e-07f) > th) {
                argmin_merge(be, bi, grey_error(kov, vR, __dsqrt_rn((double)pi.y)), pi.x * 8 + kiso);
                const float xlo = ax * (1.0f - 2.384185791015625e-07f);
                if (xlo > lb) { lb = xlo; th = flag_threshold(lb, tie_abs); }
            }
        }
    };
    build(0);
    if (lane == 0) consider(*dom0_pos, 0);
    int built = 0;
    bool overflow = false;
    for (int ch = 0; ch < n_chunks && !overflow; ch++) {
        const int64_t base = ((int64_t)ch * rows_padded + r * 8) * kFlagLists;
        const int my_cnt = lane < 8 * kFlagLists ? flag_cnt[base + lane] : 0;
        if (__any_sync(0xffffffffu, my_cnt > kFlagCap)) { overflow = true; break; }
        for (int kiso = 0; kiso < 8; kiso++) {
            int any = 0;
            for (int h = 0; h < kFlagLists; h++) any |= __shfl_sync(0xffffffffu, my_cnt, kFlagLists * kiso + h);
            if (any == 0) continue;
            if (built != kiso) { build(kiso); built = kiso; }
#pragma unroll 1
            for (int h = 0; h < kFlagLists; h++) {
                const int cnt = __shfl_sync(0xffffffffu, my_cnt, kFlagLists * kiso + h);
                if (cnt == 0) continue;
                const int2 *lst = flag_list + (base + kFlagLists * kiso + h) * kFlagCap;
                const int2 mine = lane < cnt ? lst[lane] : make_int2(0, 0);
                unsigned live = __ballot_sync(0xffffffffu, lane < cnt && __int_as_float(mine.y) > th_row);
                while (live) {
                    const int e = __ffs(live) - 1;
                    live &= live - 1;
                    consider((int64_t)__shfl_sync(0xffffffffu, mine.x, e) * 32 + lane, kiso);
                }
            }
        }
    }
    if (overflow) {
        for (int kiso = 0; kiso < 8; kiso++) {
            build(kiso);
            for (int64_t pos = lane; pos < npos; pos += 32) consider(pos, kiso);
        }
    }
    warp_argmin(be, bi);
    if (lane == 0) best[j] = bi == 0x7fffffff ? 0 : bi;
}

template <int B>
__global__ void __launch_bounds__(128)
k_umma_refine_rgb(const uint8_t *__restrict__ src, const int32_t *__restrict__ rsum, const uint8_t *__restrict__ opB,
                  const int4 *__restrict__ pos_info, const int2 *__restrict__ flag_list, const int32_t *__restrict__ flag_cnt,
                  const uint32_t *__restrict__ row_lb, int n_chunks,
                  int64_t rows_padded, int64_t rows, int64_t npos, const int64_t *__restrict__ dom0_pos,
                  int32_t *__restrict__ best, Geom g, int64_t j0)
{
    using L = Lay<B, true>;
    constexpr int n = B * B;
    const int warp = threadIdx.x >> 5, lane = threadIdx.x & 31;
    const int64_t i = (int64_t)blockIdx.x * 4 + warp;
    if (i >= rows) return;
    const int64_t j = j0 + i;
    int rm[3];
    const int vRi = centred_sum_rgb(rsum, g.NR, j, n, rm);
    const int rmsum = rm[0] + rm[1] + rm[2];
    if (vRi == 0) {
        if (lane == 0) best[j] = 0;
        return;
    }
    const float vR = (float)vRi;
    const int xr = (int)(j % g.rpw), yr = (int)(j / g.rpw);
    const int64_t plane = (int64_t)g.W * g.H;
    __shared__ float s_gR[4][n];
    float *gR = s_gR[warp];
    for (int k = lane; k < n; k += 32) {
        const uint8_t *q = src + (int64_t)(yr * B + k / B) * g.W + xr * B + (k % B);
        gR[k] = (float)((int)__ldg(q) + (int)__ldg(q + plane) + (int)__ldg(q + 2 * plane) - rmsum);
    }
    __syncwarp();
    float be = 10000000.0f;
    int bi = 0x7fffffff;
    const float tie_abs = (float)(vRi * vRi) * 4.76837158203125e-07f;
    float lb = __uint_as_float(row_lb[i]), th = lb > 0.0f ? flag_threshold(lb, tie_abs) : -1.0f;
    const float th_row = th;
    auto consider = [&](int64_t pos) {
        const int4 pi = __ldg(pos_info + pos);
        const int idx = pi.x;
        if (idx >= 0) {
            const int row = (int)(pos % kTileN);
            uint8_t *const blob = const_cast<uint8_t *>(opB) + (pos / kTileN) * L::B_TILE_BYTES;
            float kov = 0.0f;
#pragma unroll 8
            for (int c = 0; c < n / 8; c++) {
                const uint4 d = __ldg((const uint4 *)rgb_dom_piece<B>(blob, row, c));
                const uint32_t w[4] = {d.x, d.y, d.z, d.w};
#pragma unroll
                for (int e = 0; e < 4; e++) {
                    const float2 f = __half22float2(*(const __half2 *)&w[e]);
                    kov = rgb_kov_step(kov, gR[c * 8 + 2 * e], f.x);
                    kov = rgb_kov_step(kov, gR[c * 8 + 2 * e + 1], f.y);
                }
            }
            const float vD = (float)pi.y;
            const float ax = pi.y > 0 ? __fdiv_rn(fabsf(kov), vD) : 0.0f;
            if (ax * (1.0f + 2.384185791015625e-07f) > th) {
                argmin_merge(be, bi, rgb_error(kov, vR, vD), idx);
                const float xlo = ax * (1.0f - 2.384185791015625e-07f);
                if (xlo > lb) { lb = xlo; th = flag_threshold(lb, tie_abs); }
            }
        }
    };
    if (lane == 0) consider(*dom0_pos);
    for_each_flagged(lane, i, rows_padded, n_chunks, npos, flag_list, flag_cnt, th_row, consider);
    warp_argmin(be, bi);
    if (lane == 0) best[j] = bi == 0x7fffffff ? 0 : bi;
}


inline int64_t pad_up(int64_t v, int64_t m) { return (v + m - 1) / m * m; }
inline uint64_t gcd_u64(uint64_t a, uint64_t b) { while (b) { uint64_t t = a % b; a = b; b = t; } return a; }

struct Plan {
    int64_t rp;
    int n_sb, ntiles, n_chunks;
    uint32_t mult;
    int64_t npos;
};

inline int rows_per_sb(const Geom &g) { return (g.C == 3 && g.B == 16 ? 2 : kAccs) * kBlockM; }

inline Plan make_plan(const Geom &g, int64_t rows, int num_sms)
{
    Plan p;
    const int rows_sb = rows_per_sb(g);
    p.rp = pad_up(rows, 2 * rows_sb);
    p.n_sb = (int)(p.rp / rows_sb);
    p.ntiles = (int)((g.ND + kTileN - 1) / kTileN);
    p.npos = (int64_t)p.ntiles * kTileN;
    p.n_chunks = 1;
    const double tile_s = (g.B == 16 ? (g.C == 3 ? 2300.0 : 4650.0) : (g.B == 8 ? 1550.0 : 1400.0)) / 1.9e9;
    const double flag_s = 0.11e-9 * (g.n / 64.0) * (g.n > 64 ? 0.7 : 1.0);
    double best_cost = 0;
    for (int c = 1; c <= 8 && c <= p.ntiles; c++) {
        const int64_t units = (int64_t)p.n_sb * c;
        const int64_t waves = (units + num_sms - 1) / num_sms;
        const double tiles_per_unit = (double)((p.ntiles + c - 1) / c);
        const double flags_per_row = 2.0 * (log(2.0 * tiles_per_unit) + 0.58) + 2.0 * (c - 1) * 1.5;
        const double cost = (double)waves * tiles_per_unit * tile_s + (double)rows * flags_per_row * flag_s;
        if (c == 1 || cost < best_cost * 0.98) { best_cost = cost; p.n_chunks = c; }
    }
    const uint64_t nch = (uint64_t)p.ntiles * kChunksPerTile;
    uint64_t m = (uint64_t)((double)nch * 0.6180339887498949) | 1u;
    while (gcd_u64(m, nch) != 1) m += 2;
    p.mult = nch <= 8 ? 1u : (uint32_t)(m % nch);
    return p;
}

template <int B, bool F16>
struct OpBLayout {
    size_t off_posdom, off_posinfo, off_posraw, off_dom0, off_keys0, off_keys1, off_vals0, off_vals1, off_temp,
        temp_bytes, total;
    OpBLayout(const Geom &g, const Plan &p)
    {
        size_t o = (size_t)p.ntiles * Lay<B, F16>::B_TILE_BYTES;
        auto take = [&](size_t bytes) { size_t at = (o + 255) & ~(size_t)255; o = at + bytes; return at; };
        off_posdom = take((size_t)p.npos * 4);
        off_posinfo = take((size_t)p.npos * 16);
        off_posraw = take((size_t)p.npos * (B * B));
        off_dom0 = take(16);
        off_keys0 = take((size_t)g.ND * 4);
        off_keys1 = take((size_t)g.ND * 4);
        off_vals0 = take((size_t)g.ND * 4);
        off_vals1 = take((size_t)g.ND * 4);
        temp_bytes = sort_hist_bytes(g.ND);
        off_temp = take(temp_bytes + 256);
        total = o + 256;
    }
};

template <int B, bool F16>
struct OpALayout {
    static constexpr int kCntSlots = 4;
    size_t off_vR, off_cnt, off_list, off_lb, off_norm, total;
    explicit OpALayout(const Plan &p)
    {
        off_vR = (size_t)p.n_sb * Lay<B, F16>::A_SB_BYTES;
        off_cnt = off_vR + (size_t)p.rp * 4;
        off_list = off_cnt + (size_t)p.rp * p.n_chunks * kCntSlots * 4;
        off_lb = off_list + (size_t)p.rp * p.n_chunks * kFlagLists * kFlagCap * sizeof(int2);
        off_norm = off_lb + (size_t)p.rp * 4;
        total = off_norm + (size_t)p.rp * 4 + 1024;
    }
};

template <int B, bool F16>
size_t opA_bytes_t(const Geom &g, int64_t rows, int num_sms)
{
    return OpALayout<B, F16>(make_plan(g, rows, num_sms)).total;
}

using KernelT = void (*)(const uint8_t *, const uint8_t *, const int32_t *, const float *, int2 *, int32_t *, uint32_t *, int, int,
                         int, int, int64_t, int32_t *, int64_t, volatile int *);

template <int B, bool F16>
constexpr bool pair_capable() { return F16 || B == 16; }
template <int B, bool F16>
constexpr bool pair_default() { return pair_capable<B, F16>() && B >= 8; }

inline bool pair_launchable(KernelT kern, int smem_bytes)
{
    static std::mutex mu;
    static std::vector<std::tuple<KernelT, int, bool>> known;
    int dev = 0;
    cudaGetDevice(&dev);
    {
        std::lock_guard<std::mutex> lock(mu);
        for (const auto &k : known)
            if (std::get<0>(k) == kern && std::get<1>(k) == dev) return std::get<2>(k);
    }
    const bool ok = [&]() {
    cudaLaunchConfig_t cfg = {};
    cfg.gridDim = dim3(2);
    cfg.blockDim = dim3(kThreads);
    cfg.dynamicSmemBytes = (size_t)smem_bytes;
    cudaLaunchAttribute at[1];
    at[0].id = cudaLaunchAttributeClusterDimension;
    at[0].val.clusterDim.x = 2;
    at[0].val.clusterDim.y = 1;
    at[0].val.clusterDim.z = 1;
    cfg.attrs = at;
    cfg.numAttrs = 1;
    int n = 0;
    if (cudaOccupancyMaxActiveClusters(&n, (const void *)kern, &cfg) != cudaSuccess) {
        cudaGetLastError();
        return false;
    }
    return n >= 1;
    }();
    std::lock_guard<std::mutex> lock(mu);
    known.emplace_back(kern, dev, ok);
    return ok;
}

template <int B, bool F16>
int launch_t(const Work &w, const Geom &g, int64_t j0, int64_t j1, int num_sms, cudaStream_t s, const char **err,
             cudaEvent_t k0, cudaEvent_t k1, int pair_mode, int *pair_used, int32_t *dump, int64_t dump_ld, int *status_dev)
{
    using L = Lay<B, F16>;
    if (j1 <= j0) return 0;
    const int64_t rows = (j1 - j0) * g.n_iso;
    Plan p = make_plan(g, rows, num_sms);
    const int64_t rp = p.rp;
    uint8_t *opA = w.opA;
    const OpALayout<B, F16> la(p);
    int32_t *vR = (int32_t *)(opA + la.off_vR);
    int32_t *flag_cnt = (int32_t *)(opA + la.off_cnt);
    int2 *flag_list = (int2 *)(opA + la.off_list);
    uint32_t *row_lb = (uint32_t *)(opA + la.off_lb);
    float *row_norm = (float *)(opA + la.off_norm);
    const bool rgb = g.C == 3;
    if (rgb && !F16) { *err = "the RGB tensor path is kind::f16 only"; return -1; }
    OpBLayout<B, F16> lay(g, p);
    int32_t *pos_dom = (int32_t *)(w.opB + lay.off_posdom);
    int4 *pos_info = (int4 *)(w.opB + lay.off_posinfo);
    uint8_t *pos_raw = w.opB + lay.off_posraw;
    int64_t *dom0 = (int64_t *)(w.opB + lay.off_dom0);
    int launches = 0;
    cudaError_t ce;
    uint32_t *keys0 = (uint32_t *)(w.opB + lay.off_keys0), *keys1 = (uint32_t *)(w.opB + lay.off_keys1);
    int32_t *vals0 = (int32_t *)(w.opB + lay.off_vals0), *vals1 = (int32_t *)(w.opB + lay.off_vals1);
    if (rgb) k_umma_sortkeys_rgb<<<(unsigned)((g.ND + 255) / 256), 256, 0, s>>>(w.dsum, g.n, g.ND, keys0, vals0);
    else k_umma_sortkeys<<<(unsigned)((g.ND + 255) / 256), 256, 0, s>>>(w.dsum, w.dsq, g.n, g.ND, keys0, vals0);
    launches += 1 + launch_sort_pairs(keys0, vals0, keys1, vals1, (uint32_t *)(w.opB + lay.off_temp), g.ND, s);
    const int32_t *perm = vals1;
    if constexpr (F16) {
        if (rgb) {
            launches += launch_sum_planes(w.dec, w.dec3, g, s);
            k_umma_pack_domains_rgb<B><<<(unsigned)((p.npos + 127) / 128), 128, 0, s>>>(
                w.dec3, w.dsum, perm, w.opB, pos_dom, pos_info, dom0, g, p.ntiles, p.mult);
            k_umma_pack_ranges_rgb<B><<<(unsigned)((rp + 127) / 128), 128, 0, s>>>(w.src, w.rsum, opA, vR, B == 16 ? row_norm : nullptr, g, j0, j1, rp);
        }
    }
    if (!rgb) {
        k_umma_pack_domains<B, F16><<<(unsigned)((p.npos + 127) / 128), 128, 0, s>>>(
            w.dec, w.dsum, w.dsq, perm, w.opB, pos_dom, pos_info, pos_raw, dom0, g, p.ntiles, p.mult);
        k_umma_pack_ranges<B, F16><<<(unsigned)((rp + 127) / 128), 128, 0, s>>>(w.src, w.rsum, opA, vR, g, j0, j1, rp);
    }
    launches += 2;
    bool pair = false;
    KernelT kern = dump ? k_umma_search<B, F16, false, true> : k_umma_search<B, F16, false, false>;
    if constexpr (pair_capable<B, F16>()) {
        pair = (pair_mode == FIC_UMMA_PAIR_ON || (pair_mode != FIC_UMMA_PAIR_OFF && pair_default<B, F16>())) && num_sms >= 2;
        if (pair) {
            KernelT pk = dump ? k_umma_search<B, F16, true, true> : k_umma_search<B, F16, true, false>;
            ce = cudaFuncSetAttribute(pk, cudaFuncAttributeMaxDynamicSharedMemorySize, L::SMEM_BYTES);
            if (ce != cudaSuccess) { *err = cudaGetErrorString(ce); return -1; }
            if (pair_launchable(pk, L::SMEM_BYTES)) kern = pk;
            else pair = false;
        }
    }
    if (pair_used) *pair_used = pair ? 1 : 0;
    ce = cudaFuncSetAttribute(kern, cudaFuncAttributeMaxDynamicSharedMemorySize, L::SMEM_BYTES);
    if (ce != cudaSuccess) { *err = cudaGetErrorString(ce); return -1; }
    int n_units = pair ? (p.n_sb / 2) * p.n_chunks : p.n_sb * p.n_chunks;
    const int slots = pair ? num_sms / 2 : num_sms;
    int grid = (n_units < slots ? n_units : slots) * (pair ? 2 : 1);
    if (k0) cudaEventRecord(k0, s);
    cudaMemsetAsync(row_lb, 0, (size_t)rp * 4, s);
    {
        cudaLaunchConfig_t cfg = {};
        cfg.gridDim = dim3((unsigned)grid);
        cfg.blockDim = dim3(kThreads);
        cfg.dynamicSmemBytes = L::SMEM_BYTES;
        cfg.stream = s;
        cudaLaunchAttribute at[1];
        at[0].id = cudaLaunchAttributeClusterDimension;
        at[0].val.clusterDim.x = 2;
        at[0].val.clusterDim.y = 1;
        at[0].val.clusterDim.z = 1;
        cfg.attrs = at;
        cfg.numAttrs = pair ? 1 : 0;
        const uint8_t *opA_c = opA, *opB_c = w.opB;
        const int32_t *vR_c = vR;
        const float *norm_c = row_norm;
        const int iso_shift = g.n_iso > 1 ? 3 : 0;
        volatile int *status_v = status_dev;
        ce = cudaLaunchKernelEx(&cfg, kern, opA_c, opB_c, vR_c, norm_c, flag_list, flag_cnt, row_lb, p.n_sb, p.n_chunks, p.ntiles, iso_shift,
                                rp, dump, dump_ld, status_v);
        if (ce != cudaSuccess) { *err = cudaGetErrorString(ce); return -1; }
    }
    if (k1) cudaEventRecord(k1, s);
    if (rgb) {
        if constexpr (F16)
            k_umma_refine_rgb<B><<<(unsigned)((rows + 3) / 4), 128, 0, s>>>(w.src, w.rsum, w.opB, pos_info, flag_list, flag_cnt,
                                                                            row_lb, p.n_chunks, rp, rows, p.npos, dom0, w.best, g, j0);
    } else if (g.n_iso > 1)
        k_umma_refine_iso<B><<<(unsigned)((j1 - j0 + 3) / 4), 128, 0, s>>>(w.src, w.rsum, pos_raw, pos_info, flag_list, flag_cnt,
                                                                         row_lb, p.n_chunks, rp, j1 - j0, p.npos, dom0, w.best, g, j0);
    else
        k_umma_refine<B><<<(unsigned)((rows + 3) / 4), 128, 0, s>>>(w.src, w.rsum, pos_raw, pos_info, flag_list, flag_cnt,
                                                                    row_lb, p.n_chunks, rp, rows, p.npos, dom0, w.best, g, j0);
    launches += 2;
    ce = cudaGetLastError();
    if (ce != cudaSuccess) { *err = cudaGetErrorString(ce); return -1; }
    return launches;
}

#define FIC_UMMA_DISPATCH(B_, F_, EXPR_I8_4, EXPR_I8_8, EXPR_I8_16, EXPR_F16_4, EXPR_F16_8, EXPR_F16_16) \
    ((B_) == 16 ? ((F_) ? (EXPR_F16_16) : (EXPR_I8_16)) : ((F_) ? ((B_) == 8 ? (EXPR_F16_8) : (EXPR_F16_4)) : ((B_) == 8 ? (EXPR_I8_8) : (EXPR_I8_4))))

}

int umma_default_kind(const Geom &g) { return g.B == 16 ? FIC_UMMA_KIND_I8 : FIC_UMMA_KIND_F16; }

static bool use_f16(const Geom &g, int kind)
{
    if (g.C == 3) return true;
    if (g.B == 16) return false;
    return (kind == FIC_UMMA_KIND_AUTO ? umma_default_kind(g) : kind) == FIC_UMMA_KIND_F16;
}

void umma_debug_positions(const Work &w, const Geom &g, int64_t rows, int num_sms, int kind, const int32_t **d_pos_dom,
                          int64_t *npos)
{
    Plan p = make_plan(g, rows, num_sms);
    *npos = p.npos;
    const size_t off = FIC_UMMA_DISPATCH(g.B, use_f16(g, kind), (OpBLayout<4, false>(g, p).off_posdom),
                                         (OpBLayout<8, false>(g, p).off_posdom), (OpBLayout<16, false>(g, p).off_posdom),
                                         (OpBLayout<4, true>(g, p).off_posdom), (OpBLayout<8, true>(g, p).off_posdom),
                                         (OpBLayout<16, true>(g, p).off_posdom));
    *d_pos_dom = (const int32_t *)(w.opB + off);
}

double measure_mma_peak(int num_sms, cudaStream_t s, int reps, int f16, int n_cols, const char **err)
{
    const int smem = 200 * 1024;
    void (*kern)(int, uint32_t) = f16 ? (n_cols == 128 ? k_mma_peak<true, 128> : k_mma_peak<true, 256>)
                                      : (n_cols == 128 ? k_mma_peak<false, 128> : k_mma_peak<false, 256>);
    cudaError_t ce = cudaFuncSetAttribute(kern, cudaFuncAttributeMaxDynamicSharedMemorySize, smem);
    if (ce != cudaSuccess) { *err = cudaGetErrorString(ce); return -1.0; }
    cudaEvent_t e0, e1;
    cudaEventCreate(&e0);
    cudaEventCreate(&e1);
    const int iters = 200000 * 256 / n_cols;
    const double k_per_mma = f16 ? 16.0 : 32.0;
    double best = 0.0;
    for (int r = 0; r < reps + 1; r++) {
        cudaEventRecord(e0, s);
        kern<<<num_sms, 128, smem, s>>>(iters, 0x9e3779b9u + r);
        cudaEventRecord(e1, s);
        ce = cudaStreamSynchronize(s);
        if (ce != cudaSuccess) { *err = cudaGetErrorString(ce); best = -1.0; break; }
        float ms = 0;
        cudaEventElapsedTime(&ms, e0, e1);
        double tops = 2.0 * 128.0 * (double)n_cols * k_per_mma * (double)iters * num_sms / (ms * 1e-3) / 1e12;
        if (r > 0 && tops > best) best = tops;
    }
    cudaEventDestroy(e0);
    cudaEventDestroy(e1);
    return best;
}


namespace {

__global__ void k_umma_selftest_check(const uint8_t *__restrict__ src, const uint8_t *__restrict__ dec,
                                      const int32_t *__restrict__ rsum, const int32_t *__restrict__ dsum,
                                      const int32_t *__restrict__ pos_dom, const int32_t *__restrict__ dump, int64_t dump_ld,
                                      int64_t npos, Geom g, unsigned int *__restrict__ bad)
{
    const int64_t t = (int64_t)blockIdx.x * blockDim.x + threadIdx.x;
    if (t >= g.NR * npos) return;
    const int64_t i = t / npos, pos = t % npos;
    const int j = pos_dom[pos];
    if (j < 0) return;
    const int B = g.B, n = g.n;
    int rmean = 0, dmean = 0, vd = 0;
    for (int c = 0; c < g.C; c++) {
        int rm, dm;
        centred_sum(rsum[(int64_t)c * g.NR + i], n, &rm);
        vd += centred_sum(dsum[(int64_t)c * g.ND + j], n, &dm);
        rmean += rm;
        dmean += dm;
    }
    const uint8_t *r = src + (int64_t)((i / g.rpw) * B) * g.W + (i % g.rpw) * B;
    const uint8_t *d = dec + (int64_t)((j / g.dpw) * g.step) * g.sw + (j % g.dpw) * g.step;
    const int64_t rplane = (int64_t)g.W * g.H, dplane = (int64_t)g.sw * g.sh;
    int kov = 0;
    for (int k = 0; k < n; k++) {
        int rv = -rmean, dv = -dmean;
        for (int c = 0; c < g.C; c++) {
            rv += (int)r[c * rplane + (int64_t)(k / B) * g.W + k % B];
            dv += (int)d[c * dplane + (int64_t)(k / B) * g.sw + k % B];
        }
        kov += rv * dv;
    }
    if (g.C == 3 && vd == 0) kov = 0;
    if (dump[i * dump_ld + pos] != kov) atomicAdd(bad, 1u);
}

}

int umma_f16_selftest(int num_sms, cudaStream_t s, const char **err)
{
    const int W = 128, B = 8;
    Geom g, g3;
    if (make_geom(W, W, B, 2 * (W / B) - 3, FIC_MODE_GREY, &g, err) || make_geom(W, W, B, 2 * (W / B) - 3, FIC_MODE_RGB, &g3, err))
        return -1;
    std::vector<uint8_t> img((size_t)W * W);
    for (int y = 0; y < W; y++)
        for (int x = 0; x < W; x++) {
            uint32_t hpix = (uint32_t)(y * W + x) * 2654435761u;
            hpix ^= hpix >> 15; hpix *= 0x2c1b3c6du; hpix ^= hpix >> 12;
            uint32_t hcell = (uint32_t)((y / 4) * W + x / 4) * 2246822519u;
            hcell ^= hcell >> 13; hcell *= 0x9e3779b1u; hcell ^= hcell >> 16;
            int v;
            if (y < 64 && x < 64) v = (hcell >> 31) ? 255 : 0;
            else if (y < 64) v = (int)(hpix >> 24);
            else if (x < 64) v = (hpix >> 31) ? 255 : 0;
            else v = (3 * x + 2 * y + (int)(hpix >> 29)) & 255;
            img[(size_t)y * W + x] = (uint8_t)v;
        }
    Work w;
    Plan p = make_plan(g, g.NR, num_sms);
    const int64_t dump_ld = p.npos;
    int32_t *dump = nullptr;
    unsigned int *bad = nullptr;
    cudaError_t ce = cudaSuccess;
    auto alloc = [&](void **ptr, size_t bytes) { if (ce == cudaSuccess) ce = cudaMalloc(ptr, bytes); };
    alloc((void **)&w.src, 3 * (size_t)W * W);
    alloc((void **)&w.dec, 3 * (size_t)g.sw * g.sh);
    alloc((void **)&w.dec3, 2 * (size_t)g.sw * g.sh);
    alloc((void **)&w.dsum, 3 * 4 * g.ND);
    alloc((void **)&w.dsq, 3 * 4 * g.ND);
    alloc((void **)&w.rsum, 3 * 4 * g.NR);
    alloc((void **)&w.best, 4 * g.NR);
    alloc((void **)&w.opA, opA_bytes_t<8, true>(g, g.NR, num_sms));
    alloc((void **)&w.opB, OpBLayout<8, true>(g, p).total);
    alloc((void **)&dump, (size_t)p.rp * dump_ld * 4);
    alloc((void **)&bad, 4);
    int result = -1;
    if (ce == cudaSuccess) {
        for (int c = 0; c < 3; c++) cudaMemcpyAsync(w.src + (size_t)c * W * W, img.data(), img.size(), cudaMemcpyHostToDevice, s);
        cudaMemsetAsync(bad, 0, 4, s);
        bool launched = true;
        for (const Geom *gp : {(const Geom *)&g, (const Geom *)&g3}) {
            cudaMemsetAsync(dump, 0x7f, (size_t)p.rp * dump_ld * 4, s);
            launch_decimate(w.src, w.dec, *gp, s);
            launch_domain_stats(w.dec, w.dsum, w.dsq, *gp, s);
            launch_range_stats(w.src, w.rsum, *gp, s);
            if (launch_t<8, true>(w, *gp, 0, gp->NR, num_sms, s, err, nullptr, nullptr, FIC_UMMA_PAIR_AUTO, nullptr, dump, dump_ld,
                                  nullptr) < 0) {
                launched = false;
                break;
            }
            const int64_t total = gp->NR * p.npos;
            k_umma_selftest_check<<<(unsigned)((total + 255) / 256), 256, 0, s>>>(
                w.src, w.dec, w.rsum, w.dsum, (const int32_t *)(w.opB + OpBLayout<8, true>(g, p).off_posdom), dump, dump_ld,
                p.npos, *gp, bad);
        }
        if (launched) {
            unsigned int hbad = 1;
            ce = cudaMemcpyAsync(&hbad, bad, 4, cudaMemcpyDeviceToHost, s);
            if (ce == cudaSuccess) ce = cudaStreamSynchronize(s);
            if (ce == cudaSuccess) result = hbad == 0 ? 1 : 0;
        }
    }
    if (ce != cudaSuccess) { *err = cudaGetErrorString(ce); result = -1; }
    for (void *ptr : {(void *)w.src, (void *)w.dec, (void *)w.dec3, (void *)w.dsum, (void *)w.dsq, (void *)w.rsum, (void *)w.best, (void *)w.opA,
                      (void *)w.opB, (void *)dump, (void *)bad})
        if (ptr) cudaFree(ptr);
    return result;
}

int umma_debug_sort(uint32_t *d_keys, int32_t *d_vals, uint32_t *d_keys_out, int32_t *d_vals_out, int64_t n, cudaStream_t s)
{
    uint32_t *hist = nullptr;
    cudaError_t ce = cudaMalloc((void **)&hist, sort_hist_bytes(n) + 256);
    if (ce != cudaSuccess) return (int)ce;
    launch_sort_pairs(d_keys, d_vals, d_keys_out, d_vals_out, hist, n, s);
    ce = cudaStreamSynchronize(s);
    cudaFree(hist);
    return (int)ce;
}

double measure_mma_peak_pair(int num_sms, cudaStream_t s, int reps, int f16, uint32_t *tmem_bases, const char **err)
{
    const int smem = 200 * 1024;
    void (*kern)(int, uint32_t, uint32_t *) = f16 ? k_mma_peak_pair<true> : k_mma_peak_pair<false>;
    cudaError_t ce = cudaFuncSetAttribute(kern, cudaFuncAttributeMaxDynamicSharedMemorySize, smem);
    if (ce != cudaSuccess) { *err = cudaGetErrorString(ce); return -1.0; }
    uint32_t *d_out = nullptr;
    if (cudaMalloc((void **)&d_out, 4 * (size_t)num_sms) != cudaSuccess) { *err = "cudaMalloc"; return -1.0; }
    cudaEvent_t e0, e1;
    cudaEventCreate(&e0);
    cudaEventCreate(&e1);
    const int iters = 200000 * 2;
    const double k_per_mma = f16 ? 16.0 : 32.0;
    const int grid = num_sms / 2 * 2;
    double best = 0.0;
    for (int r = 0; r < reps + 1; r++) {
        cudaLaunchConfig_t cfg = {};
        cfg.gridDim = dim3((unsigned)grid);
        cfg.blockDim = dim3(128);
        cfg.dynamicSmemBytes = smem;
        cfg.stream = s;
        cudaLaunchAttribute at[1];
        at[0].id = cudaLaunchAttributeClusterDimension;
        at[0].val.clusterDim.x = 2;
        at[0].val.clusterDim.y = 1;
        at[0].val.clusterDim.z = 1;
        cfg.attrs = at;
        cfg.numAttrs = 1;
        cudaEventRecord(e0, s);
        ce = cudaLaunchKernelEx(&cfg, kern, iters, (uint32_t)(0x9e3779b9u + r), d_out);
        cudaEventRecord(e1, s);
        if (ce == cudaSuccess) ce = cudaStreamSynchronize(s);
        if (ce != cudaSuccess) { *err = cudaGetErrorString(ce); best = -1.0; break; }
        float ms = 0;
        cudaEventElapsedTime(&ms, e0, e1);
        double tops = 2.0 * 256.0 * 128.0 * k_per_mma * (double)iters * (grid / 2) / (ms * 1e-3) / 1e12;
        if (r > 0 && tops > best) best = tops;
    }
    if (tmem_bases && best >= 0.0) cudaMemcpy(tmem_bases, d_out, 16, cudaMemcpyDeviceToHost);
    cudaFree(d_out);
    cudaEventDestroy(e0);
    cudaEventDestroy(e1);
    return best;
}

bool umma_applicable(const Geom &g)
{
    if (g.wk != g.dpw || g.wk != g.dph) return false;
    if (g.C == 3) return g.n_iso == 1 && (g.B == 4 || g.B == 8 || g.B == 16);
    return g.B == 4 || g.B == 8 || g.B == 16;
}

size_t umma_opA_bytes(const Geom &g, int64_t j0, int64_t j1, int num_sms, int kind)
{
    const int64_t rows = (j1 - j0) * g.n_iso;
    return FIC_UMMA_DISPATCH(g.B, use_f16(g, kind), (opA_bytes_t<4, false>(g, rows, num_sms)),
                             (opA_bytes_t<8, false>(g, rows, num_sms)), (opA_bytes_t<16, false>(g, rows, num_sms)),
                             (opA_bytes_t<4, true>(g, rows, num_sms)), (opA_bytes_t<8, true>(g, rows, num_sms)),
                             (opA_bytes_t<16, true>(g, rows, num_sms)));
}

size_t umma_opB_bytes(const Geom &g, int kind)
{
    Plan p = make_plan(g, rows_per_sb(g), 148);
    return FIC_UMMA_DISPATCH(g.B, use_f16(g, kind), (OpBLayout<4, false>(g, p).total), (OpBLayout<8, false>(g, p).total),
                             (OpBLayout<16, false>(g, p).total), (OpBLayout<4, true>(g, p).total),
                             (OpBLayout<8, true>(g, p).total), (OpBLayout<16, true>(g, p).total));
}

int launch_search_umma(const Work &w, const Geom &g, int64_t j0, int64_t j1, int num_sms, cudaStream_t s,
                       const char **err, int kind, cudaEvent_t k0, cudaEvent_t k1, int pair, int *pair_used,
                       int32_t *dump, int64_t dump_ld, int *status_dev)
{
#define FIC_UMMA_ARGS w, g, j0, j1, num_sms, s, err, k0, k1, pair, pair_used, dump, dump_ld, status_dev
    return FIC_UMMA_DISPATCH(g.B, use_f16(g, kind), (launch_t<4, false>(FIC_UMMA_ARGS)), (launch_t<8, false>(FIC_UMMA_ARGS)),
                             (launch_t<16, false>(FIC_UMMA_ARGS)), (launch_t<4, true>(FIC_UMMA_ARGS)),
                             (launch_t<8, true>(FIC_UMMA_ARGS)), (launch_t<16, true>(FIC_UMMA_ARGS)));
#undef FIC_UMMA_ARGS
}

}
```

Before: 13400.

## Compact flat range rows and balance UMMA search work with contiguous per-slot schedule

Adds a compaction kernel that drops ranges with zero centred variance, assigning them best=0 directly, and packs only live ranges into operand A via a row_of indirection. The search kernel uses this live count to bound its work. It also replaces the strided unit/chunk loop with a Sched object that gives each SM a contiguous span of (superblock, tile) work, rotating the tile start order and tracking flag-list sets. The intent is to skip wasted MMA and epilogue work on flat blocks and to balance load across SMs. The cost is extra indirection, an extra launch and atomic, and more complex flag-set bookkeeping.

```diff
diff --git a/fractal-image-compression_b200/csrc/fic_search_umma.cu b/fractal-image-compression_b200/csrc/fic_search_umma.cu
--- a/fractal-image-compression_b200/csrc/fic_search_umma.cu
+++ b/fractal-image-compression_b200/csrc/fic_search_umma.cu
@@ -1,5 +1,6 @@
 #include <cuda_fp16.h>
 
+#include <algorithm>
 #include <cmath>
 #include <mutex>
 #include <tuple>
@@ -425,10 +426,37 @@
     if (threadIdx.x == 0) *(uint4 *)(blob + L::B_OP_BYTES + kChunksPerTile * 8) = make_uint4((uint32_t)tile_has_l, 0, 0, 0);
 }
 
+__global__ void __launch_bounds__(256)
+k_umma_compact_rows(const int32_t *__restrict__ rsum, Geom g, int64_t j0, int64_t j1, int keep_all, int32_t *__restrict__ row_of,
+                    int32_t *__restrict__ n_live, int32_t *__restrict__ best)
+{
+    const int64_t i = (int64_t)blockIdx.x * blockDim.x + threadIdx.x;
+    const int64_t j = j0 + i;
+    bool live = false;
+    if (j < j1) {
+        int m[3];
+        const int vR = g.C == 3 ? centred_sum_rgb(rsum, g.NR, j, g.n, m) : centred_sum(rsum[j], g.n, m);
+        if (vR == 0) best[j] = 0;
+        live = keep_all || vR != 0;
+    }
+    if (keep_all) {
+        if (live) row_of[i] = (int32_t)j;
+        if (i == 0) *n_live = (int32_t)(j1 - j0);
+        return;
+    }
+    const int lane = threadIdx.x & 31;
+    const unsigned mask = __ballot_sync(0xffffffffu, live);
+    int base = 0;
+    if (lane == 0 && mask) base = atomicAdd(n_live, __popc(mask));
+    base = __shfl_sync(0xffffffffu, base, 0);
+    if (live) row_of[base + __popc(mask & ((1u << lane) - 1u))] = (int32_t)j;
+}
+
 template <int B, bool F16>
 __global__ void __launch_bounds__(128)
-k_umma_pack_ranges(const uint8_t *__restrict__ src, const int32_t *__restrict__ rsum, uint8_t *__restrict__ opA,
-                   int32_t *__restrict__ vRout, Geom g, int64_t j0, int64_t j1, int64_t rows_padded)
+k_umma_pack_ranges(const uint8_t *__restrict__ src, const int32_t *__restrict__ rsum, const int32_t *__restrict__ row_of,
+                   const int32_t *__restrict__ n_live, uint8_t *__restrict__ opA, int32_t *__restrict__ vRout, Geom g,
+                   int64_t rows_padded)
 {
     using L = Lay<B, F16>;
     constexpr int n = Cfg<B, F16>::n;
@@ -439,14 +467,15 @@
     int blk = rr / kBlockM, row = rr % kBlockM;
     uint8_t *rowp = opA + sb * L::A_SB_BYTES + blk * L::A_BLOCK_BYTES + (row >> 3) * L::SBO_A + (row & 7) * 16;
     constexpr int NCH = Cfg<B, F16>::KS_A * 2;
-    const int64_t j = j0 + i / g.n_iso;
+    const int64_t blk_i = i / g.n_iso;
     const int kiso = (int)(i % g.n_iso);
-    if (j >= j1) {
+    if (blk_i >= *n_live) {
 #pragma unroll
         for (int c = 0; c < NCH; c++) *(uint4 *)(rowp + c * 128) = make_uint4(0, 0, 0, 0);
         vRout[i] = 0;
         return;
     }
+    const int64_t j = row_of[blk_i];
     int xr = (int)(j % g.rpw), yr = (int)(j / g.rpw);
     const uint8_t *p = src + (int64_t)(yr * B) * g.W + xr * B;
     int rmean;
@@ -600,8 +629,9 @@
 
 template <int B>
 __global__ void __launch_bounds__(128)
-k_umma_pack_ranges_rgb(const uint8_t *__restrict__ src, const int32_t *__restrict__ rsum, uint8_t *__restrict__ opA,
-                       int32_t *__restrict__ vRout, float *__restrict__ nRout, Geom g, int64_t j0, int64_t j1, int64_t rows_padded)
+k_umma_pack_ranges_rgb(const uint8_t *__restrict__ src, const int32_t *__restrict__ rsum, const int32_t *__restrict__ row_of,
+                       const int32_t *__restrict__ n_live, uint8_t *__restrict__ opA, int32_t *__restrict__ vRout,
+                       float *__restrict__ nRout, Geom g, int64_t rows_padded)
 {
     using L = Lay<B, true>;
     constexpr int n = B * B;
@@ -612,14 +642,14 @@
     int blk = rr / kBlockM, row = rr % kBlockM;
     uint8_t *rowp = opA + sb * L::A_SB_BYTES + blk * L::A_BLOCK_BYTES + (row >> 3) * L::SBO_A + (row & 7) * 16;
     constexpr int NCH = n / 8;
-    const int64_t j = j0 + i;
-    if (j >= j1) {
+    if (i >= *n_live) {
 #pragma unroll
         for (int c = 0; c < NCH; c++) *(uint4 *)(rowp + c * 128) = make_uint4(0, 0, 0, 0);
         vRout[i] = 0;
         if (nRout) nRout[i] = 0.0f;
         return;
     }
+    const int64_t j = row_of[i];
     const int xr = (int)(j % g.rpw), yr = (int)(j / g.rpw);
     const int64_t plane = (int64_t)g.W * g.H;
     const uint8_t *p = src + (int64_t)(yr * B) * g.W + xr * B;
@@ -831,11 +861,43 @@
 template <int B, bool F16, bool PAIR>
 __host__ __device__ constexpr int epi_of() { return (!F16 || B == 16) ? 0 : ((B == 4 || PAIR) ? 3 : 2); }
 
+struct Sched {
+    int64_t lo, e, hi, S;
+    int T, slot;
+    __device__ Sched(int slot_, int slots, int64_t P, int T_, int n_sets) : T(T_), slot(slot_)
+    {
+        const int64_t W = P * T;
+        if (n_sets == 1) S = (int64_t)T * ((P + slots - 1) / slots);
+        else {
+            S = (W + slots - 1) / slots;
+            const int64_t s_min = (T + n_sets - 2) / (n_sets - 1);
+            if (S < s_min) S = s_min;
+        }
+        lo = (int64_t)slot * S;
+        e = lo + S < W ? lo + S : W;
+        hi = e;
+    }
+    __device__ bool next(int &unit, int &t0, int &t1, int &ts, int &set)
+    {
+        if (e <= lo) return false;
+        const int64_t a = (e - 1) / T, s0 = a * T > lo ? a * T : lo;
+        unit = (int)a;
+        t0 = (int)(s0 - a * T);
+        t1 = (int)(e - a * T);
+        const int64_t len = t1 - t0, rot = ((hi - e - t0) % len + len) % len;
+        ts = t0 + (int)rot;
+        set = slot - (int)(a * T / S);
+        e = s0;
+        return true;
+    }
+};
+
 template <int B, bool F16, bool PAIR, bool DUMP>
 __global__ void __launch_bounds__(kThreads, 1)
 k_umma_search(const uint8_t *__restrict__ opA, const uint8_t *__restrict__ opB, const int32_t *__restrict__ vRarr,
-              const float *__restrict__ nRarr, int2 *__restrict__ flag_list, int32_t *__restrict__ flag_cnt, uint32_t *__restrict__ row_lb, int n_sb,
-              int n_chunks, int ntiles, int iso_shift, int64_t rows_padded, int32_t *__restrict__ dump, int64_t dump_ld, volatile int *status)
+              const float *__restrict__ nRarr, int2 *__restrict__ flag_list, int32_t *__restrict__ flag_cnt, uint32_t *__restrict__ row_lb,
+              const int32_t *__restrict__ n_live, int n_sb, int n_chunks, int ntiles, int iso_shift, int64_t rows_padded,
+              int32_t *__restrict__ dump, int64_t dump_ld, volatile int *status)
 {
     using C = Cfg<B, F16>;
     using L = Lay<B, F16>;
@@ -863,8 +925,9 @@
 
     const int warp = threadIdx.x >> 5, lane = threadIdx.x & 31;
     const uint32_t rank = PAIR ? cluster_ctarank() : 0u;
-    const int u_first = PAIR ? (int)(blockIdx.x >> 1) : (int)blockIdx.x, u_step = PAIR ? (int)(gridDim.x >> 1) : (int)gridDim.x;
-    const int n_sbu = PAIR ? (n_sb >> 1) : n_sb;
+    const int slot = PAIR ? (int)(blockIdx.x >> 1) : (int)blockIdx.x, slots = PAIR ? (int)(gridDim.x >> 1) : (int)gridDim.x;
+    const int64_t live_sb = ((int64_t)__ldg(n_live) * (1 << iso_shift) + L::ROWS_SB - 1) / L::ROWS_SB;
+    const int64_t n_work = min((int64_t)(PAIR ? n_sb >> 1 : n_sb), PAIR ? (live_sb + 1) >> 1 : live_sb);
 
     if (warp == 1 && lane == 0) {
         const uint32_t both = (PAIR && rank == 0) ? 2u : 1u;
@@ -895,18 +958,16 @@
     tc_fence_after();
     const uint32_t tmem_base = *tmem_slot;
 
-    const int n_units = n_sbu * n_chunks;
-
     if (warp == 0) {
         if (lane == 0) {
             uint32_t stage = 0, phase = 0, a_phase = 0;
-            for (int u = u_first; u < n_units; u += u_step) {
-                int sb = PAIR ? 2 * (u % n_sbu) + (int)rank : u % n_sbu, ch = u / n_sbu;
-                int t0 = (int)((int64_t)ch * ntiles / n_chunks), t1 = (int)((int64_t)(ch + 1) * ntiles / n_chunks);
+            Sched sch(slot, slots, n_work, ntiles, n_chunks);
+            for (int unit, t0, t1, ts, set; sch.next(unit, t0, t1, ts, set);) {
+                const int sb = PAIR ? 2 * unit + (int)rank : unit;
                 mbar_wait(BAR_A_EMPTY, a_phase ^ 1, status, 1);
                 mbar_expect_tx(BAR_A_FULL, L::A_SB_BYTES);
                 bulk_g2s(smem_u32(sA), opA + (int64_t)sb * L::A_SB_BYTES, L::A_SB_BYTES, BAR_A_FULL);
-                for (int t = t0; t < t1; t++) {
+                for (int k = t0, t = ts; k < t1; k++, t = t + 1 < t1 ? t + 1 : t0) {
                     const uint8_t *blob = opB + (int64_t)t * L::B_TILE_BYTES;
                     if (C::KSPLIT && PAIR) {
                         const uint32_t has_l = __ldg((const uint32_t *)(blob + L::B_OP_BYTES + kChunksPerTile * 8));
@@ -955,11 +1016,10 @@
                 uint32_t stage = 0, phase = 0, a_phase = 0, t_phase = 0;
                 const uint32_t elected = elect_one();
                 const uint64_t a_desc0 = make_desc(smem_u32(sA), 128, L::SBO_A);
-                for (int u = u_first; u < n_units; u += u_step) {
-                    int ch = u / n_sbu;
-                    int t0 = (int)((int64_t)ch * ntiles / n_chunks), t1 = (int)((int64_t)(ch + 1) * ntiles / n_chunks);
+                Sched sch(slot, slots, n_work, ntiles, n_chunks);
+                for (int unit, t0, t1, ts, set; sch.next(unit, t0, t1, ts, set);) {
                     mbar_wait(BAR_A_FULL, a_phase, status, 3);
-                    for (int t = t0; t < t1; t++) {
+                    for (int k = t0, t = ts; k < t1; k++, t = t + 1 < t1 ? t + 1 : t0) {
                         mbar_wait(BAR_B_FULL(stage), phase, status, 4);
                         tc_fence_after();
                         const uint32_t has_l = lds_volatile_u32(s_has_l + 4u * stage);
@@ -1014,12 +1074,11 @@
                 if (lane == 0) {
                     uint32_t stage = 0, phase = 0, a_phase = 0;
                     const uint32_t ra_full = mapa_u32(BAR_A_FULL, 0);
-                    for (int u = u_first; u < n_units; u += u_step) {
-                        int ch = u / n_sbu;
-                        int t0 = (int)((int64_t)ch * ntiles / n_chunks), t1 = (int)((int64_t)(ch + 1) * ntiles / n_chunks);
+                    Sched sch(slot, slots, n_work, ntiles, n_chunks);
+                    for (int unit, t0, t1, ts, set; sch.next(unit, t0, t1, ts, set);) {
                         mbar_wait(BAR_A_FULL, a_phase, status, 3);
                         mbar_arrive_cluster(ra_full);
-                        for (int t = t0; t < t1; t++) {
+                        for (int k = t0, t = ts; k < t1; k++, t = t + 1 < t1 ? t + 1 : t0) {
                             mbar_wait(BAR_B_FULL(stage), phase, status, 4);
                             const uint32_t has_l = lds_volatile_u32(s_has_l + 4u * stage);
                             mbar_arrive_cluster(mapa_u32(BAR_B_FULL(stage), 0));
@@ -1042,11 +1101,10 @@
                 const uint32_t elected = elect_one();
                 const uint64_t a_desc0 = make_desc(smem_u32(sA), 128, L::SBO_A);
                 const uint64_t b_desc0 = make_desc(smem_u32(sB), 128, L::SBO_B);
-                for (int u = u_first; u < n_units; u += u_step) {
-                    int ch = u / n_sbu;
-                    int t0 = (int)((int64_t)ch * ntiles / n_chunks), t1 = (int)((int64_t)(ch + 1) * ntiles / n_chunks);
+                Sched sch(slot, slots, n_work, ntiles, n_chunks);
+                for (int unit, t0, t1, ts, set; sch.next(unit, t0, t1, ts, set);) {
                     mbar_wait(BAR_A_FULL, a_phase, status, 3);
-                    for (int t = t0; t < t1; t++) {
+                    for (int k = t0, t = ts; k < t1; k++, t = t + 1 < t1 ? t + 1 : t0) {
                         mbar_wait(BAR_B_FULL(stage), phase, status, 4);
                         tc_fence_after();
                         const uint64_t b_desc = b_desc0 + (uint64_t)((stage * SLOT) >> 4);
@@ -1077,12 +1135,11 @@
                 if (lane == 0) {
                     uint32_t stage = 0, phase = 0, a_phase = 0;
                     const uint32_t ra_full = mapa_u32(BAR_A_FULL, 0);
-                    for (int u = u_first; u < n_units; u += u_step) {
-                        int ch = u / n_sbu;
-                        int t0 = (int)((int64_t)ch * ntiles / n_chunks), t1 = (int)((int64_t)(ch + 1) * ntiles / n_chunks);
+                    Sched sch(slot, slots, n_work, ntiles, n_chunks);
+                    for (int unit, t0, t1, ts, set; sch.next(unit, t0, t1, ts, set);) {
                         mbar_wait(BAR_A_FULL, a_phase, status, 3);
                         mbar_arrive_cluster(ra_full);
-                        for (int t = t0; t < t1; t++) {
+                        for (int k = t0, t = ts; k < t1; k++, t = t + 1 < t1 ? t + 1 : t0) {
                             mbar_wait(BAR_B_FULL(stage), phase, status, 4);
                             mbar_arrive_cluster(mapa_u32(BAR_B_FULL(stage), 0));
                             if (++stage == NSTAGE) { stage = 0; phase ^= 1; }
@@ -1098,11 +1155,10 @@
         const uint32_t elected = elect_one();
         const uint64_t a_desc0 = make_desc(smem_u32(sA), 128, L::SBO_A);
         const uint64_t b_desc0 = make_desc(smem_u32(sB), 128, L::SBO_B);
-        for (int u = u_first; u < n_units; u += u_step) {
-            int ch = u / n_sbu;
-            int t0 = (int)((int64_t)ch * ntiles / n_chunks), t1 = (int)((int64_t)(ch + 1) * ntiles / n_chunks);
+        Sched sch(slot, slots, n_work, ntiles, n_chunks);
+        for (int unit, t0, t1, ts, set; sch.next(unit, t0, t1, ts, set);) {
             mbar_wait(BAR_A_FULL, a_phase, status, 3);
-            for (int t = t0; t < t1; t++) {
+            for (int k = t0, t = ts; k < t1; k++, t = t + 1 < t1 ? t + 1 : t0) {
                 mbar_wait(BAR_B_FULL(stage), phase, status, 4);
                 tc_fence_after();
                 const uint32_t has_l = *(volatile const uint32_t *)(sB + stage * L::SLOT_BYTES + L::B_OP_BYTES + kChunksPerTile * 8);
@@ -1189,10 +1245,9 @@
             else mbar_arrive(bar_hand_back);
         };
         constexpr bool SLACK = B == 16 && F16;
-        const int n_units_mine = q < C::NB ? n_units : 0;
-        for (int u = u_first; u < n_units_mine; u += u_step) {
-            int sb = PAIR ? 2 * (u % n_sbu) + (int)rank : u % n_sbu, ch = u / n_sbu;
-            int t0 = (int)((int64_t)ch * ntiles / n_chunks), t1 = (int)((int64_t)(ch + 1) * ntiles / n_chunks);
+        Sched sch(slot, slots, q < C::NB ? n_work : 0, ntiles, n_chunks);
+        for (int unit, t0, t1, ts, set; sch.next(unit, t0, t1, ts, set);) {
+            const int sb = PAIR ? 2 * unit + (int)rank : unit;
             const int64_t row = (int64_t)sb * L::ROWS_SB + q * kBlockM + lq * 32 + lane;
             const int vR = vRarr[row];
             const float nR = SLACK ? nRarr[row] : 0.0f;
@@ -1206,16 +1261,16 @@
                 sts_u32(sh_lb, 0u);
                 __syncwarp();
             }
-            if (ch > 0 && vR != 0) {
+            if (vR != 0) {
                 const float seed = __uint_as_float(*(volatile const uint32_t *)(row_lb + ((row >> iso_shift) << iso_shift)));
                 if (seed > 0.0f) {
                     st.lbmax = seed;
                     st.thresh = flag_threshold(seed, tie_abs);
                 }
             }
-            int2 *const list0 = flag_list + (((int64_t)ch * rows_padded + row) * kFlagLists) * kFlagCap;
+            int2 *const list0 = flag_list + (((int64_t)set * rows_padded + row) * kFlagLists) * kFlagCap;
             int cnt0 = 0, cnt1 = 0;
-            for (int t = t0; t < t1; t++) {
+            for (int k = t0, t = ts; k < t1; k++, t = t + 1 < t1 ? t + 1 : t0) {
                 const float4 *gb = (const float4 *)(opB + (int64_t)t * L::B_TILE_BYTES + L::B_OP_BYTES);
                 const float4 bnd01 = __ldg(gb), bnd23 = __ldg(gb + 1);
                 float4 bndn = make_float4(0.0f, 0.0f, 0.0f, 0.0f);
@@ -1350,8 +1405,10 @@
                 }
                 tf_phase ^= 1;
             }
-            flag_cnt[((int64_t)ch * rows_padded + row) * 2] = cnt0;
-            flag_cnt[((int64_t)ch * rows_padded + row) * 2 + 1] = cnt1;
+            flag_cnt[((int64_t)set * rows_padded + row) * 2] = cnt0;
+            flag_cnt[((int64_t)set * rows_padded + row) * 2 + 1] = cnt1;
+            if (t1 == ntiles)
+                for (int s = set + 1; s < n_chunks; s++) *(int2 *)(flag_cnt + ((int64_t)s * rows_padded + row) * 2) = make_int2(0, 0);
             if (st.lbmax > 0.0f) atomicMax(row_lb + ((row >> iso_shift) << iso_shift), __float_as_uint(st.lbmax));
         }
     }
@@ -1532,16 +1589,16 @@
 k_umma_refine(const uint8_t *__restrict__ src, const int32_t *__restrict__ rsum, const uint8_t *__restrict__ pos_raw,
               const int4 *__restrict__ pos_info,
               const int2 *__restrict__ flag_list, const int32_t *__restrict__ flag_cnt,
-              const uint32_t *__restrict__ row_lb, int n_chunks,
-              int64_t rows_padded, int64_t rows, int64_t npos, const int64_t *__restrict__ dom0_pos,
-              int32_t *__restrict__ best, Geom g, int64_t j0)
+              const uint32_t *__restrict__ row_lb, const int32_t *__restrict__ row_of, const int32_t *__restrict__ n_live,
+              int n_chunks, int64_t rows_padded, int64_t npos, const int64_t *__restrict__ dom0_pos,
+              int32_t *__restrict__ best, Geom g)
 {
     constexpr int n = B * B;
     constexpr int NW = n / 4;
     const int warp = threadIdx.x >> 5, lane = threadIdx.x & 31;
     const int64_t i = (int64_t)blockIdx.x * 4 + warp;
-    if (i >= rows) return;
-    const int64_t j = j0 + i;
+    if (i >= *n_live) return;
+    const int64_t j = row_of[i];
     int rmean;
     const int vR = centred_sum(rsum[j], n, &rmean);
     if (vR == 0) {
@@ -1597,17 +1654,17 @@
 __global__ void __launch_bounds__(128)
 k_umma_refine_iso(const uint8_t *__restrict__ src, const int32_t *__restrict__ rsum, const uint8_t *__restrict__ pos_raw,
                   const int4 *__restrict__ pos_info, const int2 *__restrict__ flag_list,
-                  const int32_t *__restrict__ flag_cnt, const uint32_t *__restrict__ row_lb, int n_chunks,
-                  int64_t rows_padded, int64_t ranges, int64_t npos,
-                  const int64_t *__restrict__ dom0_pos, int32_t *__restrict__ best, Geom g, int64_t j0)
+                  const int32_t *__restrict__ flag_cnt, const uint32_t *__restrict__ row_lb, const int32_t *__restrict__ row_of,
+                  const int32_t *__restrict__ n_live, int n_chunks, int64_t rows_padded, int64_t npos,
+                  const int64_t *__restrict__ dom0_pos, int32_t *__restrict__ best, Geom g)
 {
     constexpr int n = B * B;
     constexpr int NW = n / 4;
     __shared__ uint8_t s_blk[4][n];
     const int warp = threadIdx.x >> 5, lane = threadIdx.x & 31;
     const int64_t r = (int64_t)blockIdx.x * 4 + warp;
-    if (r >= ranges) return;
-    const int64_t j = j0 + r;
+    if (r >= *n_live) return;
+    const int64_t j = row_of[r];
     int rmean;
     const int vR = centred_sum(rsum[j], n, &rmean);
     if (vR == 0) {
@@ -1694,16 +1751,16 @@
 __global__ void __launch_bounds__(128)
 k_umma_refine_rgb(const uint8_t *__restrict__ src, const int32_t *__restrict__ rsum, const uint8_t *__restrict__ opB,
                   const int4 *__restrict__ pos_info, const int2 *__restrict__ flag_list, const int32_t *__restrict__ flag_cnt,
-                  const uint32_t *__restrict__ row_lb, int n_chunks,
-                  int64_t rows_padded, int64_t rows, int64_t npos, const int64_t *__restrict__ dom0_pos,
-                  int32_t *__restrict__ best, Geom g, int64_t j0)
+                  const uint32_t *__restrict__ row_lb, const int32_t *__restrict__ row_of, const int32_t *__restrict__ n_live,
+                  int n_chunks, int64_t rows_padded, int64_t npos, const int64_t *__restrict__ dom0_pos,
+                  int32_t *__restrict__ best, Geom g)
 {
     using L = Lay<B, true>;
     constexpr int n = B * B;
     const int warp = threadIdx.x >> 5, lane = threadIdx.x & 31;
     const int64_t i = (int64_t)blockIdx.x * 4 + warp;
-    if (i >= rows) return;
-    const int64_t j = j0 + i;
+    if (i >= *n_live) return;
+    const int64_t j = row_of[i];
     int rm[3];
     const int vRi = centred_sum_rgb(rsum, g.NR, j, n, rm);
     const int rmsum = rm[0] + rm[1] + rm[2];
@@ -1772,7 +1829,7 @@
 
 inline int rows_per_sb(const Geom &g) { return (g.C == 3 && g.B == 16 ? 2 : kAccs) * kBlockM; }
 
-inline Plan make_plan(const Geom &g, int64_t rows, int num_sms)
+inline Plan make_plan(const Geom &g, int64_t rows, int num_sms, bool pair)
 {
     Plan p;
     const int rows_sb = rows_per_sb(g);
@@ -1784,12 +1841,13 @@
     const double tile_s = (g.B == 16 ? (g.C == 3 ? 2300.0 : 4650.0) : (g.B == 8 ? 1550.0 : 1400.0)) / 1.9e9;
     const double flag_s = 0.11e-9 * (g.n / 64.0) * (g.n > 64 ? 0.7 : 1.0);
     double best_cost = 0;
+    const int64_t units = pair ? p.n_sb / 2 : p.n_sb, slots = pair ? num_sms / 2 : num_sms;
     for (int c = 1; c <= 8 && c <= p.ntiles; c++) {
-        const int64_t units = (int64_t)p.n_sb * c;
-        const int64_t waves = (units + num_sms - 1) / num_sms;
+        const int64_t share = c == 1 ? p.ntiles * ((units + slots - 1) / slots)
+                                     : std::max((units * p.ntiles + slots - 1) / slots, (int64_t)(p.ntiles + c - 2) / (c - 1));
         const double tiles_per_unit = (double)((p.ntiles + c - 1) / c);
         const double flags_per_row = 2.0 * (log(2.0 * tiles_per_unit) + 0.58) + 2.0 * (c - 1) * 1.5;
-        const double cost = (double)waves * tiles_per_unit * tile_s + (double)rows * flags_per_row * flag_s;
+        const double cost = (double)share * tile_s + (double)rows * flags_per_row * flag_s;
         if (c == 1 || cost < best_cost * 0.98) { best_cost = cost; p.n_chunks = c; }
     }
     const uint64_t nch = (uint64_t)p.ntiles * kChunksPerTile;
@@ -1824,26 +1882,28 @@
 template <int B, bool F16>
 struct OpALayout {
     static constexpr int kCntSlots = 4;
-    size_t off_vR, off_cnt, off_list, off_lb, off_norm, total;
+    size_t off_vR, off_cnt, off_list, off_lb, off_live, off_norm, off_rowof, total;
     explicit OpALayout(const Plan &p)
     {
         off_vR = (size_t)p.n_sb * Lay<B, F16>::A_SB_BYTES;
         off_cnt = off_vR + (size_t)p.rp * 4;
         off_list = off_cnt + (size_t)p.rp * p.n_chunks * kCntSlots * 4;
         off_lb = off_list + (size_t)p.rp * p.n_chunks * kFlagLists * kFlagCap * sizeof(int2);
-        off_norm = off_lb + (size_t)p.rp * 4;
-        total = off_norm + (size_t)p.rp * 4 + 1024;
+        off_live = off_lb + (size_t)p.rp * 4;
+        off_norm = off_live + 16;
+        off_rowof = off_norm + (size_t)p.rp * 4;
+        total = off_rowof + (size_t)p.rp * 4 + 1024;
     }
 };
 
 template <int B, bool F16>
 size_t opA_bytes_t(const Geom &g, int64_t rows, int num_sms)
 {
-    return OpALayout<B, F16>(make_plan(g, rows, num_sms)).total;
-}
-
-using KernelT = void (*)(const uint8_t *, const uint8_t *, const int32_t *, const float *, int2 *, int32_t *, uint32_t *, int, int,
-                         int, int, int64_t, int32_t *, int64_t, volatile int *);
+    return std::max(OpALayout<B, F16>(make_plan(g, rows, num_sms, false)).total, OpALayout<B, F16>(make_plan(g, rows, num_sms, true)).total);
+}
+
+using KernelT = void (*)(const uint8_t *, const uint8_t *, const int32_t *, const float *, int2 *, int32_t *, uint32_t *,
+                         const int32_t *, int, int, int, int, int64_t, int32_t *, int64_t, volatile int *);
 
 template <int B, bool F16>
 constexpr bool pair_capable() { return F16 || B == 16; }
@@ -1892,44 +1952,9 @@
     using L = Lay<B, F16>;
     if (j1 <= j0) return 0;
     const int64_t rows = (j1 - j0) * g.n_iso;
-    Plan p = make_plan(g, rows, num_sms);
-    const int64_t rp = p.rp;
-    uint8_t *opA = w.opA;
-    const OpALayout<B, F16> la(p);
-    int32_t *vR = (int32_t *)(opA + la.off_vR);
-    int32_t *flag_cnt = (int32_t *)(opA + la.off_cnt);
-    int2 *flag_list = (int2 *)(opA + la.off_list);
-    uint32_t *row_lb = (uint32_t *)(opA + la.off_lb);
-    float *row_norm = (float *)(opA + la.off_norm);
     const bool rgb = g.C == 3;
     if (rgb && !F16) { *err = "the RGB tensor path is kind::f16 only"; return -1; }
-    OpBLayout<B, F16> lay(g, p);
-    int32_t *pos_dom = (int32_t *)(w.opB + lay.off_posdom);
-    int4 *pos_info = (int4 *)(w.opB + lay.off_posinfo);
-    uint8_t *pos_raw = w.opB + lay.off_posraw;
-    int64_t *dom0 = (int64_t *)(w.opB + lay.off_dom0);
-    int launches = 0;
     cudaError_t ce;
-    uint32_t *keys0 = (uint32_t *)(w.opB + lay.off_keys0), *keys1 = (uint32_t *)(w.opB + lay.off_keys1);
-    int32_t *vals0 = (int32_t *)(w.opB + lay.off_vals0), *vals1 = (int32_t *)(w.opB + lay.off_vals1);
-    if (rgb) k_umma_sortkeys_rgb<<<(unsigned)((g.ND + 255) / 256), 256, 0, s>>>(w.dsum, g.n, g.ND, keys0, vals0);
-    else k_umma_sortkeys<<<(unsigned)((g.ND + 255) / 256), 256, 0, s>>>(w.dsum, w.dsq, g.n, g.ND, keys0, vals0);
-    launches += 1 + launch_sort_pairs(keys0, vals0, keys1, vals1, (uint32_t *)(w.opB + lay.off_temp), g.ND, s);
-    const int32_t *perm = vals1;
-    if constexpr (F16) {
-        if (rgb) {
-            launches += launch_sum_planes(w.dec, w.dec3, g, s);
-            k_umma_pack_domains_rgb<B><<<(unsigned)((p.npos + 127) / 128), 128, 0, s>>>(
-                w.dec3, w.dsum, perm, w.opB, pos_dom, pos_info, dom0, g, p.ntiles, p.mult);
-            k_umma_pack_ranges_rgb<B><<<(unsigned)((rp + 127) / 128), 128, 0, s>>>(w.src, w.rsum, opA, vR, B == 16 ? row_norm : nullptr, g, j0, j1, rp);
-        }
-    }
-    if (!rgb) {
-        k_umma_pack_domains<B, F16><<<(unsigned)((p.npos + 127) / 128), 128, 0, s>>>(
-            w.dec, w.dsum, w.dsq, perm, w.opB, pos_dom, pos_info, pos_raw, dom0, g, p.ntiles, p.mult);
-        k_umma_pack_ranges<B, F16><<<(unsigned)((rp + 127) / 128), 128, 0, s>>>(w.src, w.rsum, opA, vR, g, j0, j1, rp);
-    }
-    launches += 2;
     bool pair = false;
     KernelT kern = dump ? k_umma_search<B, F16, false, true> : k_umma_search<B, F16, false, false>;
     if constexpr (pair_capable<B, F16>()) {
@@ -1945,11 +1970,50 @@
     if (pair_used) *pair_used = pair ? 1 : 0;
     ce = cudaFuncSetAttribute(kern, cudaFuncAttributeMaxDynamicSharedMemorySize, L::SMEM_BYTES);
     if (ce != cudaSuccess) { *err = cudaGetErrorString(ce); return -1; }
-    int n_units = pair ? (p.n_sb / 2) * p.n_chunks : p.n_sb * p.n_chunks;
+    Plan p = make_plan(g, rows, num_sms, pair);
+    const int64_t rp = p.rp;
+    uint8_t *opA = w.opA;
+    const OpALayout<B, F16> la(p);
+    int32_t *vR = (int32_t *)(opA + la.off_vR);
+    int32_t *flag_cnt = (int32_t *)(opA + la.off_cnt);
+    int2 *flag_list = (int2 *)(opA + la.off_list);
+    uint32_t *row_lb = (uint32_t *)(opA + la.off_lb);
+    int32_t *n_live = (int32_t *)(opA + la.off_live);
+    float *row_norm = (float *)(opA + la.off_norm);
+    int32_t *row_of = (int32_t *)(opA + la.off_rowof);
+    OpBLayout<B, F16> lay(g, p);
+    int32_t *pos_dom = (int32_t *)(w.opB + lay.off_posdom);
+    int4 *pos_info = (int4 *)(w.opB + lay.off_posinfo);
+    uint8_t *pos_raw = w.opB + lay.off_posraw;
+    int64_t *dom0 = (int64_t *)(w.opB + lay.off_dom0);
+    int launches = 0;
+    uint32_t *keys0 = (uint32_t *)(w.opB + lay.off_keys0), *keys1 = (uint32_t *)(w.opB + lay.off_keys1);
+    int32_t *vals0 = (int32_t *)(w.opB + lay.off_vals0), *vals1 = (int32_t *)(w.opB + lay.off_vals1);
+    if (rgb) k_umma_sortkeys_rgb<<<(unsigned)((g.ND + 255) / 256), 256, 0, s>>>(w.dsum, g.n, g.ND, keys0, vals0);
+    else k_umma_sortkeys<<<(unsigned)((g.ND + 255) / 256), 256, 0, s>>>(w.dsum, w.dsq, g.n, g.ND, keys0, vals0);
+    launches += 1 + launch_sort_pairs(keys0, vals0, keys1, vals1, (uint32_t *)(w.opB + lay.off_temp), g.ND, s);
+    const int32_t *perm = vals1;
+    cudaMemsetAsync(row_lb, 0, la.off_norm - la.off_lb, s);
+    k_umma_compact_rows<<<(unsigned)((j1 - j0 + 255) / 256), 256, 0, s>>>(w.rsum, g, j0, j1, dump ? 1 : 0, row_of, n_live, w.best);
+    if constexpr (F16) {
+        if (rgb) {
+            launches += launch_sum_planes(w.dec, w.dec3, g, s);
+            k_umma_pack_domains_rgb<B><<<(unsigned)((p.npos + 127) / 128), 128, 0, s>>>(
+                w.dec3, w.dsum, perm, w.opB, pos_dom, pos_info, dom0, g, p.ntiles, p.mult);
+            k_umma_pack_ranges_rgb<B><<<(unsigned)((rp + 127) / 128), 128, 0, s>>>(w.src, w.rsum, row_of, n_live, opA, vR,
+                                                                                 B == 16 ? row_norm : nullptr, g, rp);
+        }
+    }
+    if (!rgb) {
+        k_umma_pack_domains<B, F16><<<(unsigned)((p.npos + 127) / 128), 128, 0, s>>>(
+            w.dec, w.dsum, w.dsq, perm, w.opB, pos_dom, pos_info, pos_raw, dom0, g, p.ntiles, p.mult);
+        k_umma_pack_ranges<B, F16><<<(unsigned)((rp + 127) / 128), 128, 0, s>>>(w.src, w.rsum, row_of, n_live, opA, vR, g, rp);
+    }
+    launches += 3;
+    const int64_t n_units = pair ? p.n_sb / 2 : p.n_sb;
     const int slots = pair ? num_sms / 2 : num_sms;
-    int grid = (n_units < slots ? n_units : slots) * (pair ? 2 : 1);
+    const int grid = (int)std::min<int64_t>(n_units * p.n_chunks, slots) * (pair ? 2 : 1);
     if (k0) cudaEventRecord(k0, s);
-    cudaMemsetAsync(row_lb, 0, (size_t)rp * 4, s);
     {
         cudaLaunchConfig_t cfg = {};
         cfg.gridDim = dim3((unsigned)grid);
@@ -1968,21 +2032,23 @@
         const float *norm_c = row_norm;
         const int iso_shift = g.n_iso > 1 ? 3 : 0;
         volatile int *status_v = status_dev;
-        ce = cudaLaunchKernelEx(&cfg, kern, opA_c, opB_c, vR_c, norm_c, flag_list, flag_cnt, row_lb, p.n_sb, p.n_chunks, p.ntiles, iso_shift,
-                                rp, dump, dump_ld, status_v);
+        const int32_t *live_c = n_live;
+        ce = cudaLaunchKernelEx(&cfg, kern, opA_c, opB_c, vR_c, norm_c, flag_list, flag_cnt, row_lb, live_c, p.n_sb, p.n_chunks, p.ntiles,
+                                iso_shift, rp, dump, dump_ld, status_v);
         if (ce != cudaSuccess) { *err = cudaGetErrorString(ce); return -1; }
     }
     if (k1) cudaEventRecord(k1, s);
+    const unsigned rblocks = (unsigned)((j1 - j0 + 3) / 4);
     if (rgb) {
         if constexpr (F16)
-            k_umma_refine_rgb<B><<<(unsigned)((rows + 3) / 4), 128, 0, s>>>(w.src, w.rsum, w.opB, pos_info, flag_list, flag_cnt,
-                                                                            row_lb, p.n_chunks, rp, rows, p.npos, dom0, w.best, g, j0);
+            k_umma_refine_rgb<B><<<rblocks, 128, 0, s>>>(w.src, w.rsum, w.opB, pos_info, flag_list, flag_cnt, row_lb, row_of, n_live,
+                                                         p.n_chunks, rp, p.npos, dom0, w.best, g);
     } else if (g.n_iso > 1)
-        k_umma_refine_iso<B><<<(unsigned)((j1 - j0 + 3) / 4), 128, 0, s>>>(w.src, w.rsum, pos_raw, pos_info, flag_list, flag_cnt,
-                                                                         row_lb, p.n_chunks, rp, j1 - j0, p.npos, dom0, w.best, g, j0);
+        k_umma_refine_iso<B><<<rblocks, 128, 0, s>>>(w.src, w.rsum, pos_raw, pos_info, flag_list, flag_cnt, row_lb, row_of, n_live,
+                                                     p.n_chunks, rp, p.npos, dom0, w.best, g);
     else
-        k_umma_refine<B><<<(unsigned)((rows + 3) / 4), 128, 0, s>>>(w.src, w.rsum, pos_raw, pos_info, flag_list, flag_cnt,
-                                                                    row_lb, p.n_chunks, rp, rows, p.npos, dom0, w.best, g, j0);
+        k_umma_refine<B><<<rblocks, 128, 0, s>>>(w.src, w.rsum, pos_raw, pos_info, flag_list, flag_cnt, row_lb, row_of, n_live,
+                                                 p.n_chunks, rp, p.npos, dom0, w.best, g);
     launches += 2;
     ce = cudaGetLastError();
     if (ce != cudaSuccess) { *err = cudaGetErrorString(ce); return -1; }
@@ -2006,7 +2072,7 @@
 void umma_debug_positions(const Work &w, const Geom &g, int64_t rows, int num_sms, int kind, const int32_t **d_pos_dom,
                           int64_t *npos)
 {
-    Plan p = make_plan(g, rows, num_sms);
+    Plan p = make_plan(g, rows, num_sms, false);
     *npos = p.npos;
     const size_t off = FIC_UMMA_DISPATCH(g.B, use_f16(g, kind), (OpBLayout<4, false>(g, p).off_posdom),
                                          (OpBLayout<8, false>(g, p).off_posdom), (OpBLayout<16, false>(g, p).off_posdom),
@@ -2105,7 +2171,7 @@
             img[(size_t)y * W + x] = (uint8_t)v;
         }
     Work w;
-    Plan p = make_plan(g, g.NR, num_sms);
+    Plan p = make_plan(g, g.NR, num_sms, false);
     const int64_t dump_ld = p.npos;
     int32_t *dump = nullptr;
     unsigned int *bad = nullptr;
@@ -2230,7 +2296,7 @@
 
 size_t umma_opB_bytes(const Geom &g, int kind)
 {
-    Plan p = make_plan(g, rows_per_sb(g), 148);
+    Plan p = make_plan(g, rows_per_sb(g), 148, false);
     return FIC_UMMA_DISPATCH(g.B, use_f16(g, kind), (OpBLayout<4, false>(g, p).total), (OpBLayout<8, false>(g, p).total),
                              (OpBLayout<16, false>(g, p).total), (OpBLayout<4, true>(g, p).total),
                              (OpBLayout<8, true>(g, p).total), (OpBLayout<16, true>(g, p).total));
```

After: 13390 (median of 6 runs). Within noise of the previous version (-0.1%).
